# AnyLoc/AnyLoc

Hardware: NVIDIA H100
Metric: images/sec end-to-end DINOv2-VLAD descriptors (higher is better)
Workload: dtype f32-equivalent (tensor-core fp16 3-term split, fp32 accumulate)

## Files before the change

### anyloc_b200/_lib.py

```python
import ctypes as C
import os

import torch

_HERE = os.path.dirname(os.path.abspath(__file__))
LIB_PATH = os.path.join(_HERE, "libanyloc_b200.so")

DIST = {"cosine": 0, "euclidean": 1}
METRIC = {"cosine": 0, "l2": 1}
FACET = {"query": 0, "key": 1, "value": 2, "token": 3}
FFN = {"mlp": 0, "swiglufused": 1}
EPI = {"bias": 0, "bias_split": 1, "gelu_split": 2, "swiglu_split": 3, "ls_resid": 4}
ENGINE = {"auto": 0, "simt": 1, "tc3": 2}
PAIR = {"tf32": 0, "f16": 1, "bf16": 2, "fp8": 3, "f16x1": 4}
ACT_SCALE = 8.0
VIT_VARLEN_MAX_B = 128
PREPROCESS_VARLEN_BATCH = 64
ERR = {"arg": -1, "cuda": -2, "workspace": -3, "unsupported": -4}
PCA = {"cov": 0, "gram": 1, "vt": 2, "sketch": 3}
VLAD_ROUTE_SORTED = 2
KMEANS_SMEM_BYTES = 220 * 1024


class AnylocError(RuntimeError):
    pass


class VitCfg(C.Structure):
    _fields_ = [(n, C.c_int) for n in ("embed_dim", "depth", "num_heads", "ffn_kind", "ffn_hidden", "patch",
                                       "pair_dtype", "num_registers")]


_BLOCK_FIELDS = ["ln1_w", "ln1_b", "qkv_w_hi", "qkv_w_lo", "qkv_b", "proj_w_hi", "proj_w_lo", "proj_b",
                 "ls1", "ln2_w", "ln2_b", "in_w_hi", "in_w_lo", "in_b", "out_w_hi", "out_w_lo", "out_b", "ls2"]


class VitBlock(C.Structure):
    _fields_ = [(n, C.c_void_p) for n in _BLOCK_FIELDS] + \
               [(n, C.c_float) for n in ("qkv_alpha", "proj_alpha", "in_alpha", "out_alpha")]


class VitWeightsStruct(C.Structure):
    _fields_ = [("patch_w_hi", C.c_void_p), ("patch_w_lo", C.c_void_p), ("patch_b", C.c_void_p),
                ("cls_token", C.c_void_p), ("blocks", C.POINTER(VitBlock)), ("patch_alpha", C.c_float),
                ("register_tokens", C.c_void_p)]


class VitTap(C.Structure):
    _fields_ = [("layer", C.c_int), ("facet", C.c_int), ("out", C.c_void_p)]


_SIGS = {
    "anyloc_last_error": (C.c_char_p, []),
    "anyloc_version": (C.c_int, []),
    "anyloc_launch_count": (C.c_longlong, []),
    "anyloc_profile_enable": (C.c_int, [C.c_int]),
    "anyloc_profile_read": (C.c_int, [C.POINTER(C.c_double), C.POINTER(C.c_longlong), C.POINTER(C.c_double)]),
    "anyloc_device_info": (C.c_int, [C.POINTER(C.c_int), C.POINTER(C.c_size_t)]),
    "anyloc_vlad_workspace_bytes": (C.c_size_t, [C.c_int] * 4),
    "anyloc_vlad_generate": (C.c_int, [C.c_void_p, C.c_void_p, C.c_void_p] + [C.c_int] * 7 +
                             [C.c_void_p, C.c_void_p, C.c_void_p, C.c_size_t, C.c_void_p]),
    "anyloc_vlad_prepared_bytes": (C.c_size_t, [C.c_int] * 2),
    "anyloc_vlad_prepare": (C.c_int, [C.c_void_p, C.c_int, C.c_int, C.c_int, C.c_void_p, C.c_size_t, C.c_void_p]),
    "anyloc_vlad_generate_prepared": (C.c_int, [C.c_void_p, C.c_void_p, C.c_void_p, C.c_void_p, C.c_size_t] +
                                      [C.c_int] * 7 + [C.c_void_p, C.c_void_p, C.c_void_p, C.c_size_t, C.c_void_p]),
    "anyloc_vlad_generate_route": (C.c_int, [C.c_int] * 4),
    "anyloc_vlad_sorted_workspace_bytes": (C.c_size_t, [C.c_int] * 4),
    "anyloc_vlad_generate_sorted": (C.c_int, [C.c_void_p, C.c_void_p, C.c_void_p, C.c_void_p, C.c_size_t] +
                                    [C.c_int] * 7 + [C.c_void_p, C.c_void_p, C.c_void_p, C.c_size_t, C.c_void_p]),
    "anyloc_vlad_generate_soft": (C.c_int, [C.c_void_p, C.c_void_p, C.c_void_p] + [C.c_int] * 4 + [C.c_float] +
                                  [C.c_int] * 2 + [C.c_void_p, C.c_void_p, C.c_void_p, C.c_size_t, C.c_void_p]),
    "anyloc_preprocess_u8": (C.c_int, [C.c_void_p] + [C.c_int] * 7 + [C.POINTER(C.c_float)] * 2 +
                             [C.c_void_p, C.c_void_p]),
    "anyloc_preprocess_resize_u8": (C.c_int, [C.c_void_p] + [C.c_int] * 10 + [C.POINTER(C.c_float)] * 2 +
                                    [C.c_void_p, C.c_void_p]),
    "anyloc_preprocess_u8_varlen": (C.c_int, [C.c_int, C.POINTER(C.c_void_p)] + [C.POINTER(C.c_int)] * 4 + [C.c_int] +
                                    [C.POINTER(C.c_int)] * 4 + [C.POINTER(C.c_float)] * 2 +
                                    [C.c_void_p, C.POINTER(C.c_int64), C.c_void_p]),
    "anyloc_pool": (C.c_int, [C.c_void_p, C.c_void_p] + [C.c_int] * 4 + [C.c_float, C.c_int, C.c_void_p, C.c_void_p]),
    "anyloc_vlad_residuals": (C.c_int, [C.c_void_p, C.c_void_p] + [C.c_int] * 4 + [C.c_void_p, C.c_void_p]),
    "anyloc_vlad_from_residuals_workspace_bytes": (C.c_size_t, [C.c_int] * 2),
    "anyloc_vlad_from_residuals": (C.c_int, [C.c_void_p, C.c_void_p, C.c_void_p] + [C.c_int] * 4 +
                                   [C.c_void_p, C.c_void_p, C.c_size_t, C.c_void_p]),
    "anyloc_vlad_assign": (C.c_int, [C.c_void_p, C.c_void_p] + [C.c_int] * 4 +
                           [C.c_void_p, C.c_void_p, C.c_size_t, C.c_void_p]),
    "anyloc_kmeans_workspace_bytes": (C.c_size_t, [C.c_int] * 3),
    "anyloc_kmeans_update": (C.c_int, [C.c_void_p, C.c_void_p, C.c_void_p] + [C.c_int] * 3 +
                             [C.c_void_p, C.c_void_p, C.c_void_p, C.c_size_t, C.c_void_p]),
    "anyloc_kmeans_partition": (C.c_int, [C.c_int64, C.c_int, C.POINTER(C.c_int), C.POINTER(C.c_int64)]),
    "anyloc_kmeans_round_workspace_bytes": (C.c_size_t, [C.c_int64, C.c_int, C.c_int]),
    "anyloc_kmeans_accumulate_round": (C.c_int, [C.c_void_p, C.c_void_p, C.c_int64, C.c_int64, C.c_int64, C.c_int,
                                                 C.c_int, C.c_int, C.c_void_p, C.c_size_t, C.c_void_p]),
    "anyloc_kmeans_finalize": (C.c_int, [C.c_void_p, C.c_int64, C.c_int, C.c_int, C.c_void_p, C.c_void_p, C.c_void_p,
                                         C.c_size_t, C.c_void_p]),
    "anyloc_kmeans_accumulate_round_tiled": (C.c_int, [C.c_void_p, C.c_void_p, C.c_int64, C.c_int64, C.c_int64] +
                                             [C.c_int] * 4 + [C.c_void_p, C.c_size_t, C.c_void_p]),
    "anyloc_kmeans_update_tiled": (C.c_int, [C.c_void_p, C.c_void_p, C.c_void_p, C.c_int64] + [C.c_int] * 3 +
                                   [C.c_void_p, C.c_void_p, C.c_void_p, C.c_size_t, C.c_void_p]),
    "anyloc_topk_workspace_bytes": (C.c_size_t, [C.c_int] * 4),
    "anyloc_topk": (C.c_int, [C.c_void_p, C.c_void_p] + [C.c_int] * 6 +
                    [C.c_void_p, C.c_void_p, C.c_void_p, C.c_size_t, C.c_void_p]),
    "anyloc_index_bytes": (C.c_size_t, [C.c_int64, C.c_int, C.c_int]),
    "anyloc_index_init": (C.c_int, [C.c_void_p, C.c_size_t, C.c_int64, C.c_int, C.c_int, C.c_void_p]),
    "anyloc_index_copy": (C.c_int, [C.c_void_p, C.c_size_t, C.c_int64, C.c_void_p, C.c_size_t, C.c_int64, C.c_int64,
                                    C.c_int, C.c_int, C.c_void_p]),
    "anyloc_index_add": (C.c_int, [C.c_void_p, C.c_size_t, C.c_int64, C.c_int64, C.c_void_p, C.c_int, C.c_int, C.c_int,
                                   C.c_void_p]),
    "anyloc_index_search_workspace_bytes": (C.c_size_t, [C.c_int64, C.c_int, C.c_int, C.c_int]),
    "anyloc_index_search": (C.c_int, [C.c_void_p, C.c_size_t, C.c_int64, C.c_int64, C.c_void_p] + [C.c_int] * 5 +
                            [C.c_void_p, C.c_void_p, C.c_void_p, C.c_size_t, C.c_void_p]),
    "anyloc_index_search_continue": (C.c_int, [C.c_void_p, C.c_size_t] + [C.c_int64] * 5 + [C.c_void_p] +
                                     [C.c_int] * 5 + [C.c_void_p, C.c_void_p, C.c_void_p, C.c_size_t, C.c_void_p]),
    "anyloc_index_split_bytes": (C.c_size_t, [C.c_int64, C.c_int]),
    "anyloc_index_split_init": (C.c_int, [C.c_void_p, C.c_size_t, C.c_int64, C.c_int, C.c_void_p]),
    "anyloc_index_split_copy": (C.c_int, [C.c_void_p, C.c_size_t, C.c_int64, C.c_void_p, C.c_size_t, C.c_int64,
                                          C.c_int64, C.c_int, C.c_void_p]),
    "anyloc_index_split_add": (C.c_int, [C.c_void_p, C.c_size_t, C.c_int64, C.c_void_p, C.c_int64, C.c_void_p, C.c_int,
                                         C.c_int, C.c_void_p]),
    "anyloc_index_split_search_workspace_bytes": (C.c_size_t, [C.c_int64, C.c_int, C.c_int]),
    "anyloc_index_split_stage_bytes": (C.c_size_t, [C.c_int64, C.c_int]),
    "anyloc_index_split_search": (C.c_int, [C.c_void_p, C.c_size_t, C.c_int64, C.c_int64, C.c_void_p] + [C.c_int] * 3 +
                                  [C.c_void_p, C.c_size_t, C.POINTER(C.c_int64), C.c_void_p]),
    "anyloc_index_split_rescore": (C.c_int, [C.c_void_p, C.c_size_t, C.c_int64, C.c_void_p, C.c_int64] + [C.c_int] * 3 +
                                   [C.c_void_p, C.c_size_t, C.c_int64, C.c_void_p, C.c_size_t, C.c_void_p, C.c_void_p,
                                    C.c_void_p]),
    "anyloc_index_split_piece": (C.c_int, [C.c_void_p, C.c_size_t, C.c_int64, C.c_void_p, C.c_size_t, C.c_int64,
                                           C.c_void_p, C.c_int64, C.c_int64, C.c_int, C.c_void_p]),
    "anyloc_allgather_desc": (C.c_int, [C.c_void_p, C.c_void_p, C.c_void_p, C.c_size_t, C.c_int, C.c_void_p]),
    "anyloc_vit_patch_k": (C.c_int, [C.c_int]),
    "anyloc_vit_workspace_bytes": (C.c_size_t, [C.POINTER(VitCfg), C.c_int, C.c_int, C.c_int]),
    "anyloc_vit_extract": (C.c_int, [C.POINTER(VitCfg), C.POINTER(VitWeightsStruct), C.c_void_p,
                                     C.c_int, C.c_int, C.c_int, C.c_void_p, C.c_int, C.c_int, C.c_int,
                                     C.c_int, C.c_void_p, C.c_void_p, C.c_size_t, C.c_int, C.c_void_p]),
    "anyloc_vit_varlen_workspace_bytes": (C.c_size_t, [C.POINTER(VitCfg), C.c_int, C.POINTER(C.c_int32)]),
    "anyloc_vit_extract_varlen": (C.c_int, [C.POINTER(VitCfg), C.POINTER(VitWeightsStruct), C.c_int,
                                            C.POINTER(C.c_void_p), C.POINTER(C.c_int32), C.POINTER(C.c_void_p),
                                            C.c_int, C.c_int, C.c_int, C.c_int, C.c_void_p, C.c_void_p, C.c_size_t,
                                            C.c_int, C.c_void_p]),
    "anyloc_vit_taps_workspace_bytes": (C.c_size_t, [C.POINTER(VitCfg), C.c_int, C.c_int, C.c_int, C.POINTER(VitTap),
                                                     C.c_int]),
    "anyloc_vit_extract_taps": (C.c_int, [C.POINTER(VitCfg), C.POINTER(VitWeightsStruct), C.c_void_p, C.c_int, C.c_int,
                                          C.c_int, C.c_void_p, C.POINTER(VitTap), C.c_int, C.c_int, C.c_int,
                                          C.c_void_p, C.c_size_t, C.c_int, C.c_void_p]),
    "anyloc_vit_taps_varlen_workspace_bytes": (C.c_size_t, [C.POINTER(VitCfg), C.c_int, C.POINTER(C.c_int32),
                                                            C.POINTER(VitTap), C.c_int]),
    "anyloc_vit_extract_taps_varlen": (C.c_int, [C.POINTER(VitCfg), C.POINTER(VitWeightsStruct), C.c_int,
                                                 C.POINTER(C.c_void_p), C.POINTER(C.c_int32), C.POINTER(C.c_void_p),
                                                 C.POINTER(VitTap), C.c_int, C.c_int, C.c_int, C.c_void_p, C.c_size_t,
                                                 C.c_int, C.c_void_p]),
    "anyloc_gemm_nt": (C.c_int, [C.c_void_p, C.c_void_p, C.c_int, C.c_void_p, C.c_void_p, C.c_int,
                                 C.c_int, C.c_int, C.c_int, C.c_int, C.c_float, C.c_int, C.c_void_p, C.c_void_p,
                                 C.c_void_p, C.c_void_p, C.c_void_p, C.c_int, C.c_int, C.c_int, C.c_void_p]),
    "anyloc_gemm_tc_last_staged": (C.c_int, []),
    "anyloc_split_tf32": (C.c_int, [C.c_void_p, C.c_void_p, C.c_void_p, C.c_size_t, C.c_void_p]),
    "anyloc_split_f16": (C.c_int, [C.c_void_p, C.c_void_p, C.c_void_p, C.c_size_t, C.c_float, C.c_void_p]),
    "anyloc_split_bf16": (C.c_int, [C.c_void_p, C.c_void_p, C.c_size_t, C.c_void_p]),
    "anyloc_layernorm_split": (C.c_int, [C.c_void_p, C.c_void_p, C.c_void_p, C.c_int, C.c_int, C.c_float,
                                         C.c_void_p, C.c_void_p, C.c_int, C.c_void_p]),
    "anyloc_fp8_scale": (C.c_float, [C.c_float]),
    "anyloc_quantize_fp8_rows": (C.c_int, [C.c_void_p, C.c_int, C.c_int, C.c_void_p, C.c_void_p, C.c_void_p]),
    "anyloc_quantize_fp8_tensor": (C.c_int, [C.c_void_p, C.c_void_p, C.c_size_t, C.POINTER(C.c_float), C.c_void_p]),
    "anyloc_attention": (C.c_int, [C.c_void_p, C.c_void_p, C.c_int, C.c_int, C.c_int, C.c_int, C.c_void_p,
                                   C.c_void_p, C.c_int, C.c_int, C.c_void_p]),
    "anyloc_attention_varlen": (C.c_int, [C.c_void_p, C.c_void_p, C.c_int, C.POINTER(C.c_int32),
                                          C.POINTER(C.c_int32), C.c_int, C.c_int, C.c_void_p, C.c_void_p, C.c_int,
                                          C.c_void_p]),
    "anyloc_l2_normalize_rows": (C.c_int, [C.c_void_p, C.c_int64, C.c_int, C.c_int64, C.c_void_p, C.c_void_p]),
    "anyloc_pca_colsum_workspace_bytes": (C.c_size_t, [C.c_int64, C.c_int]),
    "anyloc_pca_colsum": (C.c_int, [C.c_void_p, C.c_int64, C.c_int64, C.c_int, C.c_void_p, C.c_void_p, C.c_size_t,
                                    C.c_void_p]),
    "anyloc_pca_accumulate": (C.c_int, [C.c_int, C.c_void_p, C.c_int64, C.c_int64, C.c_int, C.c_void_p, C.c_void_p,
                                        C.c_int64, C.c_int, C.c_void_p, C.c_int64, C.c_void_p]),
    "anyloc_pca_mirror": (C.c_int, [C.c_void_p, C.c_int, C.c_int64, C.c_void_p]),
}
EXPORTS = sorted(_SIGS)

_lib = None


def load():
    global _lib
    if _lib is None:
        if not os.path.isfile(LIB_PATH):
            raise AnylocError(
                f"{LIB_PATH} is missing -- build it with `python -m anyloc_b200.build` "
                "(anyloc_b200 has no CPU fallback)")
        lib = C.CDLL(LIB_PATH)
        for name, (res, args) in _SIGS.items():
            fn = getattr(lib, name)
            fn.restype, fn.argtypes = res, args
        _lib = lib
    return _lib


def last_error():
    return load().anyloc_last_error().decode()


def check(rc, what):
    if rc != 0:
        raise AnylocError(f"{what} failed (rc={rc}): {last_error()}")


def require_cuda(device=None):
    if not torch.cuda.is_available():
        raise AnylocError("anyloc_b200 needs a CUDA device (sm_90a); there is no CPU fallback")
    load()
    dev = torch.device("cuda" if device is None else device)
    if dev.type != "cuda":
        raise AnylocError(f"anyloc_b200 runs on CUDA devices only (got device={device!r}); no CPU fallback")
    if dev.index is None:
        dev = torch.device("cuda", torch.cuda.current_device())
    return dev


def stream_ptr():
    return C.c_void_p(torch.cuda.current_stream().cuda_stream)


def ptr(t):
    if t is None:
        return C.c_void_p(0)
    assert t.is_cuda and t.is_contiguous(), "device-contiguous tensor required"
    return C.c_void_p(t.data_ptr())


class _WorkspacePool:

    def __init__(self):
        self._bufs = {}

    def get(self, device, nbytes, tag="default"):
        key = (device.index, tag)
        buf = self._bufs.get(key)
        if buf is None or buf.numel() < nbytes:
            self._bufs.pop(key, None)
            buf = None
            buf = torch.empty(int(nbytes), dtype=torch.uint8, device=device)
            self._bufs[key] = buf
        return buf

    def clear(self):
        self._bufs.clear()


workspaces = _WorkspacePool()

PROF_CATEGORIES = ["gemm_tc", "gemm_simt", "attention", "layernorm", "vit_misc", "vlad", "topk"]


def profile_enable(on=True):
    check(load().anyloc_profile_enable(int(bool(on))), "profile_enable")


def profile_read():
    n = len(PROF_CATEGORIES)
    ms, groups, work = (C.c_double * n)(), (C.c_longlong * n)(), (C.c_double * n)()
    check(load().anyloc_profile_read(ms, groups, work), "profile_read")
    return {c: (ms[i], groups[i], work[i]) for i, c in enumerate(PROF_CATEGORIES)}


def launch_count():
    return int(load().anyloc_launch_count())
```

### anyloc_b200/csrc/gemm_tc.cu

```cuda
#include <cuda.h>
#include <stdlib.h>
#include "epilogue.cuh"
#include "tc_common.cuh"

namespace anyloc {

namespace tc {

constexpr int BM = 128, BN = 128;
constexpr int KSTEPS = 4;
constexpr int A_BYTES = BM * 128;
constexpr int B_BYTES = BN * 128;
constexpr int THREADS = 384;
constexpr int STG_BYTES = 8192;

template <bool LO, bool STG = LO> struct Cfg {
  static constexpr int STAGE_BYTES = (LO ? 2 : 1) * (A_BYTES + B_BYTES);
  static constexpr int B_OFF = (LO ? 2 : 1) * A_BYTES;
  static constexpr int STAGES = LO ? 3 : 6;
  static constexpr int BAR_OFF = STAGES * STAGE_BYTES;
  static constexpr int SMEM_BYTES = BAR_OFF + 256 + 1024 ;
  static constexpr bool STAGED = STG;
  static constexpr int STG_OFF = BAR_OFF + 1024;
  static constexpr int SMEM_BYTES_STAGED = STG_OFF + 4 * STG_BYTES + 1024 ;
};
constexpr int BAND_N = 16;
constexpr int CHUNK_KB_TF32 = 2;
constexpr int CHUNK_KB_F16 = 8;
constexpr int CHUNK_KB_COARSE = 32;
constexpr int CHUNK_KB_FP8 = 1;

__device__ __forceinline__ void tile_coords(int tile, int num_m, int num_n, int band_n, int& m_blk, int& n_blk) {
  const int per_band = num_m * band_n;
  const int band = tile / per_band, r = tile - band * per_band;
  const int w = min(band_n, num_n - band * band_n);
  m_blk = r / w;
  n_blk = band * band_n + (r - m_blk * w);
}

template <int OUT>
__device__ __forceinline__ void split_put2(const EpiParams& ep, size_t o, float a, float b) {
  typedef typename Fmt<OUT>::T T;
  put2<OUT>(reinterpret_cast<T*>(ep.out), reinterpret_cast<T*>(ep.out_lo), o, a, b);
}
template <int FMT = ANYLOC_PAIR_TF32>
__device__ __forceinline__ void store_split2(const EpiParams& ep, size_t o, float a, float b) {
  if constexpr (!Fmt<FMT>::LO) split_put2<Fmt<FMT>::OUT>(ep, o, a, b);
  else if (ep.out_fmt != ANYLOC_PAIR_TF32) split_put2<ANYLOC_PAIR_F16>(ep, o, a, b);
  else split_put2<ANYLOC_PAIR_TF32>(ep, o, a, b);
}

template <int FMT = ANYLOC_PAIR_TF32>
__device__ __forceinline__ void epi_pair(const EpiParams& ep, int m, int n, int N, float v0, float v1) {
  const int mode = ep.mode;
  if (mode < 0) return;
  if (mode == ANYLOC_EPI_SWIGLU_SPLIT) {
    epi_store_pair<FMT>(ep, m, n, v0, v1);
    return;
  }
  if (n + 1 >= N || (ep.ldo & 1)) {
    epi_store1<FMT>(ep, m, n, v0);
    if (n + 1 < N) epi_store1<FMT>(ep, m, n + 1, v1);
    return;
  }
  const float al = ep.alpha;
  float2 b = make_float2(0.f, 0.f);
  if (ep.bias) b = __ldg(reinterpret_cast<const float2*>(ep.bias + n));
  const float x0 = v0 * al + b.x, x1 = v1 * al + b.y;
  const size_t o = (size_t)m * ep.ldo + n;
  if (mode == ANYLOC_EPI_BIAS) {
    *reinterpret_cast<float2*>(ep.out + o) = make_float2(x0, x1);
  } else if (mode == ANYLOC_EPI_LS_RESID) {
    const float2 g = __ldg(reinterpret_cast<const float2*>(ep.gamma + n));
    const float2 r = *reinterpret_cast<const float2*>(ep.resid + o);
    *reinterpret_cast<float2*>(ep.out + o) = make_float2(r.x + g.x * x0, r.y + g.y * x1);
  } else if (mode == ANYLOC_EPI_GELU_SPLIT) {
    store_split2<FMT>(ep, o, gelu_erf(x0), gelu_erf(x1));
  } else {
    store_split2<FMT>(ep, o, x0, x1);
  }
}

template <int FMT = ANYLOC_PAIR_TF32>
__device__ __forceinline__ void epilogue_pairs(const EpiParams& ep, int r0, int nq, int M, int N, const float* sum) {
#pragma unroll
  for (int j = 0; j < 16; ++j) {
    const int n = nq + j * 8;
    if (n >= N) continue;
    if (r0 < M) epi_pair<FMT>(ep, r0, n, N, sum[4 * j], sum[4 * j + 1]);
    if (r0 + 8 < M) epi_pair<FMT>(ep, r0 + 8, n, N, sum[4 * j + 2], sum[4 * j + 3]);
  }
}

__device__ __forceinline__ void epilogue_regs_batched(const EpiParams& ep, int r0, int nq, int M, int N, const float* sum) {
  const int mode = ep.mode;
  if (mode < 0) return;
  const int n0 = nq & ~(BN - 1);
  const bool swiglu = mode == ANYLOC_EPI_SWIGLU_SPLIT, resid = mode == ANYLOC_EPI_LS_RESID;
  if (n0 + BN > N || (!swiglu && (ep.ldo & 1))) {
    epilogue_pairs(ep, r0, nq, M, N, sum);
    return;
  }
  const bool row0 = r0 < M, row1 = r0 + 8 < M;
  const size_t o0 = (size_t)r0 * ep.ldo, o1 = (size_t)(r0 + 8) * ep.ldo;
  const float al = ep.alpha;
#pragma unroll
  for (int j0 = 0; j0 < 16; j0 += 2) {
    float2 b[2], g[2], ra[2], rb[2];
#pragma unroll
    for (int jj = 0; jj < 2; ++jj) {
      const int n = nq + (j0 + jj) * 8;
      b[jj] = ep.bias ? __ldg(reinterpret_cast<const float2*>(ep.bias + n)) : make_float2(0.f, 0.f);
      if (resid) {
        g[jj] = __ldg(reinterpret_cast<const float2*>(ep.gamma + n));
        if (row0) ra[jj] = *reinterpret_cast<const float2*>(ep.resid + o0 + n);
        if (row1) rb[jj] = *reinterpret_cast<const float2*>(ep.resid + o1 + n);
      }
    }
#pragma unroll
    for (int jj = 0; jj < 2; ++jj) {
      const int j = j0 + jj, n = nq + j * 8;
#pragma unroll
      for (int h = 0; h < 2; ++h) {
        if (!(h ? row1 : row0)) continue;
        const float v0 = sum[4 * j + 2 * h], v1 = sum[4 * j + 2 * h + 1];
        const size_t ro = h ? o1 : o0;
        if (swiglu) {
          const float x1 = v0 * al + b[jj].x, x2 = v1 * al + b[jj].y;
          epi_store_split(ep, ro + (n >> 1), silu(x1) * x2);
          continue;
        }
        const float x0 = v0 * al + b[jj].x, x1 = v1 * al + b[jj].y;
        const size_t o = ro + n;
        if (mode == ANYLOC_EPI_BIAS) {
          *reinterpret_cast<float2*>(ep.out + o) = make_float2(x0, x1);
        } else if (resid) {
          const float2 r = h ? rb[jj] : ra[jj];
          *reinterpret_cast<float2*>(ep.out + o) = make_float2(r.x + g[jj].x * x0, r.y + g[jj].y * x1);
        } else if (mode == ANYLOC_EPI_GELU_SPLIT) {
          store_split2(ep, o, gelu_erf(x0), gelu_erf(x1));
        } else {
          store_split2(ep, o, x0, x1);
        }
      }
    }
  }
}

constexpr int OUT_F32 = -1;
constexpr int STG_HALF = STG_BYTES / 2;
constexpr int STG_ROWS = 64;

template <int OUT> constexpr bool stage_lo() {
  if constexpr (OUT == OUT_F32) return false;
  else return Fmt<OUT>::LO;
}
template <int OUT> constexpr int stage_esz() {
  if constexpr (OUT == OUT_F32) return 4;
  else return (int)sizeof(typename Fmt<OUT>::T);
}
template <int OUT>
struct StageFmt {
  static constexpr bool LO = stage_lo<OUT>();
  static constexpr int ESZ = stage_esz<OUT>();
  static constexpr int ROW_BYTES = STG_BYTES / STG_ROWS / (LO ? 2 : 1);
  static constexpr int COLS = ROW_BYTES / ESZ;
  static constexpr uint32_t SWZ = ROW_BYTES == 128 ? 7 : 3;
};

template <int OUT>
__device__ __forceinline__ uint32_t stg_off(int row, int b) {
  const uint32_t o = (uint32_t)(row * StageFmt<OUT>::ROW_BYTES + b);
  return o ^ (((o >> 7) & StageFmt<OUT>::SWZ) << 4);
}

__device__ __forceinline__ float2 ldg_col_pair(const float* p, int n, int N) {
  if (n + 1 < N) return __ldg(reinterpret_cast<const float2*>(p + n));
  return make_float2(n < N ? __ldg(p + n) : 0.f, 0.f);
}

__device__ __forceinline__ void resid_load(const CUtensorMap* tm, uint8_t* buf, uint64_t* bar, int oc, int m0) {
  mbar_expect_tx(smem_u32(bar), STG_BYTES);
  tma_load_2d(smem_u32(buf), tm, smem_u32(bar), oc, m0);
}

template <int OUT, bool SWIGLU, bool RESID>
__device__ __forceinline__ void epilogue_staged(const EpiParams& ep, const CUtensorMap* tm_out, const CUtensorMap* tm_lo,
                                                const CUtensorMap* tm_resid, uint8_t* stg, uint64_t* rbar,
                                                uint32_t& rphase, uint32_t& cnt, int wg, int t, int m0, int n0, int N,
                                                const float* sum) {
  using F = StageFmt<OUT>;
  constexpr int ACC = SWIGLU ? 2 * F::COLS : F::COLS;
  constexpr int JS = ACC / 8;
  const int lane = t & 31, q = lane & 3, row = (t >> 5) * 16 + (lane >> 2);
  const int n_out = SWIGLU ? N >> 1 : N;
  const int oc_base = SWIGLU ? n0 >> 1 : n0;
  const bool gelu = ep.mode == ANYLOC_EPI_GELU_SPLIT;
  const float al = ep.alpha;
#pragma unroll
  for (int s = 0; s < BN / ACC; ++s) {
    const int oc0 = oc_base + s * F::COLS;
    if (oc0 >= n_out) break;
    const uint32_t b = cnt & 1;
    uint8_t* buf = stg + b * STG_BYTES;
    if (RESID) { mbar_wait(smem_u32(rbar + b), (rphase >> b) & 1); rphase ^= 1u << b; }
#pragma unroll
    for (int jj = 0; jj < JS; ++jj) {
      const int j = s * JS + jj, n = n0 + j * 8 + 2 * q;
      const float2 bb = ep.bias ? ldg_col_pair(ep.bias, n, N) : make_float2(0.f, 0.f);
      float2 g;
      if (RESID) g = ldg_col_pair(ep.gamma, n, N);
#pragma unroll
      for (int h = 0; h < 2; ++h) {
        const int r = row + 8 * h;
        const float x0 = sum[4 * j + 2 * h] * al + bb.x, x1 = sum[4 * j + 2 * h + 1] * al + bb.y;
        if constexpr (SWIGLU) {
          typedef typename Fmt<OUT>::T E;
          const float v = silu(x0) * x1;
          const uint32_t o = stg_off<OUT>(r, (4 * jj + q) * F::ESZ);
          E hi, lo;
          Fmt<OUT>::split1(v, hi, lo);
          *reinterpret_cast<E*>(buf + o) = hi;
          if constexpr (F::LO) *reinterpret_cast<E*>(buf + STG_HALF + o) = lo;
          continue;
        }
        const uint32_t o = stg_off<OUT>(r, (8 * jj + 2 * q) * F::ESZ);
        if constexpr (OUT == OUT_F32) {
          float2* p = reinterpret_cast<float2*>(buf + o);
          if (RESID) {
            const float2 rr = *p;
            *p = make_float2(rr.x + g.x * x0, rr.y + g.y * x1);
          } else {
            *p = make_float2(x0, x1);
          }
        } else {
          typedef typename Fmt<OUT>::W2 W;
          const float y0 = gelu ? gelu_erf(x0) : x0, y1 = gelu ? gelu_erf(x1) : x1;
          W hi, lo;
          Fmt<OUT>::split2(y0, y1, hi, lo);
          *reinterpret_cast<W*>(buf + o) = hi;
          if constexpr (F::LO) *reinterpret_cast<W*>(buf + STG_HALF + o) = lo;
        }
      }
    }
    fence_proxy_async_smem();
    if (t == 0) bulk_wait_read<0>();
    if (wg == 1) named_bar_sync<1>(128);
    else named_bar_sync<2>(128);
    if (t == 0) {
      tma_store_2d(tm_out, smem_u32(buf), oc0, m0);
      if (F::LO) tma_store_2d(tm_lo, smem_u32(buf + STG_HALF), oc0, m0);
      bulk_commit();
      if (RESID && s + 2 < BN / ACC && oc0 + 2 * F::COLS < n_out) {
        bulk_wait_read<0>();
        resid_load(tm_resid, buf, rbar + b, oc0 + 2 * F::COLS, m0);
      }
    }
    ++cnt;
  }
}

template <int FMT, int LOM>
__global__ void __launch_bounds__(THREADS, 1)
gemm_tc3_kernel(const __grid_constant__ CUtensorMap tm_a_hi, const __grid_constant__ CUtensorMap tm_a_lo,
                const __grid_constant__ CUtensorMap tm_b_hi, const __grid_constant__ CUtensorMap tm_b_lo,
                const __grid_constant__ CUtensorMap tm_out, const __grid_constant__ CUtensorMap tm_out_lo,
                const __grid_constant__ CUtensorMap tm_resid, int staged,
                int M, int N, int K, int band_n, int chunk_kb, EpiParams ep) {
  constexpr bool LO = LOM != 0, has_a_lo = (LOM & 1) != 0, has_b_lo = (LOM & 2) != 0;
  static_assert(LOM == 0 || Fmt<FMT>::LO, "lo operands belong to the pair formats");
  using C = Cfg<LO, LO || !Fmt<FMT>::LO>;
  if (ep.gate != nullptr && *reinterpret_cast<const volatile int*>(ep.gate) == 0) return;
  extern __shared__ uint8_t smem_raw[];
  uint8_t* smem = reinterpret_cast<uint8_t*>((reinterpret_cast<uintptr_t>(smem_raw) + 1023) & ~(uintptr_t)1023);
  uint64_t* full_bar = reinterpret_cast<uint64_t*>(smem + C::BAR_OFF);
  uint64_t* empty_bar = full_bar + C::STAGES;
  uint64_t* resid_bar = empty_bar + C::STAGES;

  const int wg = threadIdx.x >> 7;
  const int num_m = (M + BM - 1) / BM, num_n = (N + BN - 1) / BN;
  const int num_tiles = num_m * num_n;
  constexpr int BKE = 128 / (int)sizeof(typename Fmt<FMT>::T);
  const int num_k = (K + BKE - 1) / BKE;

  if (threadIdx.x == 0) {
    asm volatile("prefetch.tensormap [%0];" ::"l"(&tm_a_hi) : "memory");
    asm volatile("prefetch.tensormap [%0];" ::"l"(&tm_b_hi) : "memory");
    for (int s = 0; s < C::STAGES; ++s) { mbar_init(smem_u32(full_bar + s), 1); mbar_init(smem_u32(empty_bar + s), 2); }
    if (C::STAGED)
      for (int i = 0; i < 4; ++i) mbar_init(smem_u32(resid_bar + i), 1);
    asm volatile("fence.mbarrier_init.release.cluster;" ::: "memory");
  }
  __syncthreads();

  if (wg == 0) {
    if (threadIdx.x == 0) {
      const uint32_t tx_bytes = A_BYTES * (1 + ((LO && has_a_lo) ? 1 : 0)) + B_BYTES * (1 + ((LO && has_b_lo) ? 1 : 0));
      int stage = 0; uint32_t phase = 0;
      for (int tile = blockIdx.x; tile < num_tiles; tile += gridDim.x) {
        int mb, nb; tile_coords(tile, num_m, num_n, band_n, mb, nb);
        const int m0 = mb * BM, n0 = nb * BN;
        for (int kb = 0; kb < num_k; ++kb) {
          mbar_wait(smem_u32(empty_bar + stage), phase ^ 1);
          const uint32_t fb = smem_u32(full_bar + stage);
          mbar_expect_tx(fb, tx_bytes);
          const uint32_t sbase = smem_u32(smem + stage * C::STAGE_BYTES);
          tma_load_2d(sbase, &tm_a_hi, fb, kb * BKE, m0);
          if (LO && has_a_lo) tma_load_2d(sbase + A_BYTES, &tm_a_lo, fb, kb * BKE, m0);
          tma_load_2d(sbase + C::B_OFF, &tm_b_hi, fb, kb * BKE, n0);
          if (LO && has_b_lo) tma_load_2d(sbase + C::B_OFF + B_BYTES, &tm_b_lo, fb, kb * BKE, n0);
          if (++stage == C::STAGES) { stage = 0; phase ^= 1; }
        }
      }
    }
    return;
  }

  const int t = threadIdx.x & 127, warp = t >> 5, lane = t & 31;
  const uint32_t a_sub = (uint32_t)(wg - 1) * 64 * 128;
  uint8_t* stg = smem + C::STG_OFF + (wg - 1) * 2 * STG_BYTES;
  uint64_t* rbar = resid_bar + (wg - 1) * 2;
  const int mode = ep.mode;
  staged = C::STAGED && staged;
  const bool resid_staged = staged && mode == ANYLOC_EPI_LS_RESID;
  uint32_t stg_cnt = 0, rphase = 0;
  int stage = 0; uint32_t phase = 0;
  for (int tile = blockIdx.x; tile < num_tiles; tile += gridDim.x) {
    int mb, nb; tile_coords(tile, num_m, num_n, band_n, mb, nb);
    const int m0 = mb * BM + (wg - 1) * 64, n0 = nb * BN;
    float sum[64], acc[64];
#pragma unroll
    for (int j = 0; j < 64; ++j) { sum[j] = 0.f; acc[j] = 0.f; }
    int prev_stage = -1;
    for (int kb0 = 0; kb0 < num_k; kb0 += chunk_kb) {
      const int kb1 = min(num_k, kb0 + chunk_kb);
      if (resid_staged && kb1 == num_k && t == 0 && m0 < M) {
        bulk_wait_read<0>();
        for (int i = 0; i < 2; ++i) {
          const uint32_t b = (stg_cnt + i) & 1;
          const int oc = n0 + i * StageFmt<OUT_F32>::COLS;
          if (oc < N) resid_load(&tm_resid, stg + b * STG_BYTES, rbar + b, oc, m0);
        }
      }
      for (int kb = kb0; kb < kb1; ++kb) {
        mbar_wait(smem_u32(full_bar + stage), phase);
        const uint32_t sbase = smem_u32(smem + stage * C::STAGE_BYTES);
        const uint64_t a_hi = make_desc(sbase + a_sub), a_lo = make_desc(sbase + A_BYTES + a_sub);
        const uint64_t b_hi = make_desc(sbase + C::B_OFF), b_lo = make_desc(sbase + C::B_OFF + B_BYTES);
        wgmma_fence();
#pragma unroll
        for (int k = 0; k < KSTEPS; ++k) {
          const uint64_t adv = (uint64_t)((k * 32) >> 4);
          wgmma_m64n128<FMT>(acc, a_hi + adv, b_hi + adv, (kb != kb0 || k != 0) ? 1u : 0u);
          if (has_a_lo) wgmma_m64n128<FMT>(acc, a_lo + adv, b_hi + adv, 1u);
          if (has_b_lo) wgmma_m64n128<FMT>(acc, a_hi + adv, b_lo + adv, 1u);
        }
        wgmma_commit();
        wgmma_wait<1>();
        if (prev_stage >= 0 && t == 0) mbar_arrive(smem_u32(empty_bar + prev_stage));
        prev_stage = stage;
        if (++stage == C::STAGES) { stage = 0; phase ^= 1; }
      }
      wgmma_wait<0>();
      fence_regs<64>(acc);
#pragma unroll
      for (int j = 0; j < 64; ++j) sum[j] += acc[j];
    }
    if (t == 0) mbar_arrive(smem_u32(empty_bar + prev_stage));
    if (mode < 0 || m0 >= M) continue;
    if constexpr (FMT == ANYLOC_PAIR_FP8) {
      const int r = m0 + warp * 16 + (lane >> 2);
      const float s0 = r < M ? __ldg(ep.row_scale + r) : 0.f, s1 = r + 8 < M ? __ldg(ep.row_scale + r + 8) : 0.f;
#pragma unroll
      for (int j = 0; j < 16; ++j) { sum[4 * j] *= s0; sum[4 * j + 1] *= s0; sum[4 * j + 2] *= s1; sum[4 * j + 3] *= s1; }
    }
    if constexpr (!C::STAGED) {
      epilogue_regs_batched(ep, m0 + warp * 16 + (lane >> 2), n0 + 2 * (lane & 3), M, N, sum);
      continue;
    }
    if (!staged) {
      epilogue_pairs<FMT>(ep, m0 + warp * 16 + (lane >> 2), n0 + 2 * (lane & 3), M, N, sum);
      continue;
    }
#define ANYLOC_EPI_STAGED(OUT_, SWIGLU_, RESID_)                                                                    \
  epilogue_staged<OUT_, SWIGLU_, RESID_>(ep, &tm_out, &tm_out_lo, &tm_resid, stg, rbar, rphase, stg_cnt, wg, t, m0,  \
                                         n0, N, sum)
    if (mode == ANYLOC_EPI_BIAS) ANYLOC_EPI_STAGED(OUT_F32, false, false);
    else if (mode == ANYLOC_EPI_LS_RESID) ANYLOC_EPI_STAGED(OUT_F32, false, true);
    else if constexpr (!Fmt<FMT>::LO) {
      if (mode == ANYLOC_EPI_SWIGLU_SPLIT) ANYLOC_EPI_STAGED(Fmt<FMT>::OUT, true, false);
      else ANYLOC_EPI_STAGED(Fmt<FMT>::OUT, false, false);
    } else if (mode == ANYLOC_EPI_SWIGLU_SPLIT) {
      if (ep.out_fmt != ANYLOC_PAIR_TF32) ANYLOC_EPI_STAGED(ANYLOC_PAIR_F16, true, false);
      else ANYLOC_EPI_STAGED(ANYLOC_PAIR_TF32, true, false);
    } else {
      if (ep.out_fmt != ANYLOC_PAIR_TF32) ANYLOC_EPI_STAGED(ANYLOC_PAIR_F16, false, false);
      else ANYLOC_EPI_STAGED(ANYLOC_PAIR_TF32, false, false);
    }
#undef ANYLOC_EPI_STAGED
  }
  if (staged && t == 0) bulk_wait<0>();
}

typedef CUresult (*EncodeTiledFn)(CUtensorMap*, CUtensorMapDataType, cuuint32_t, void*, const cuuint64_t*,
                                  const cuuint64_t*, const cuuint32_t*, const cuuint32_t*, CUtensorMapInterleave,
                                  CUtensorMapSwizzle, CUtensorMapL2promotion, CUtensorMapFloatOOBfill);

static EncodeTiledFn get_encode() {
  static EncodeTiledFn fn = nullptr;
  if (!fn) {
    void* p = nullptr;
    cudaDriverEntryPointQueryResult q;
    if (cudaGetDriverEntryPoint("cuTensorMapEncodeTiled", &p, cudaEnableDefault, &q) != cudaSuccess ||
        q != cudaDriverEntryPointSuccess)
      return nullptr;
    fn = (EncodeTiledFn)p;
  }
  return fn;
}

static CUtensorMapDataType map_dtype(int fmt) {
  switch (fmt) {
    case ANYLOC_PAIR_FP8: return CU_TENSOR_MAP_DATA_TYPE_UINT8;
    case ANYLOC_PAIR_BF16: return CU_TENSOR_MAP_DATA_TYPE_BFLOAT16;
    case ANYLOC_PAIR_F16: case ANYLOC_PAIR_F16X1: return CU_TENSOR_MAP_DATA_TYPE_FLOAT16;
    default: return CU_TENSOR_MAP_DATA_TYPE_FLOAT32;
  }
}

int make_map(CUtensorMap* map, const void* ptr, int rows, int K, int ld, int box_rows, int fmt) {
  EncodeTiledFn enc = get_encode();
  if (!enc) { set_error("gemm_tc: cuTensorMapEncodeTiled unavailable"); return ANYLOC_ERR_CUDA; }
  const int esz = format_info(fmt).esz;
  cuuint64_t dims[2] = {(cuuint64_t)K, (cuuint64_t)rows};
  cuuint64_t strides[1] = {(cuuint64_t)ld * esz};
  cuuint32_t box[2] = {(cuuint32_t)(128 / esz), (cuuint32_t)box_rows};
  cuuint32_t estr[2] = {1, 1};
  CUresult r = enc(map, map_dtype(fmt), 2, (void*)ptr, dims, strides, box, estr, CU_TENSOR_MAP_INTERLEAVE_NONE, CU_TENSOR_MAP_SWIZZLE_128B,
                   CU_TENSOR_MAP_L2_PROMOTION_L2_256B, CU_TENSOR_MAP_FLOAT_OOB_FILL_NONE);
  if (r != CUDA_SUCCESS) { set_error("gemm_tc: cuTensorMapEncodeTiled failed (%d) rows=%d K=%d ld=%d", (int)r, rows, K, ld); return ANYLOC_ERR_CUDA; }
  return ANYLOC_OK;
}

int make_map_3d16(CUtensorMap* map, const void* ptr, int imgs, int rows, int cols, int box_rows, int fmt) {
  EncodeTiledFn enc = get_encode();
  if (!enc) { set_error("tensor map: cuTensorMapEncodeTiled unavailable"); return ANYLOC_ERR_CUDA; }
  cuuint64_t dims[3] = {(cuuint64_t)cols, (cuuint64_t)rows, (cuuint64_t)imgs};
  cuuint64_t strides[2] = {(cuuint64_t)cols * 2, (cuuint64_t)rows * cols * 2};
  cuuint32_t box[3] = {64, (cuuint32_t)box_rows, 1};
  cuuint32_t estr[3] = {1, 1, 1};
  CUresult r = enc(map, map_dtype(fmt), 3, (void*)ptr, dims,
                   strides, box, estr, CU_TENSOR_MAP_INTERLEAVE_NONE, CU_TENSOR_MAP_SWIZZLE_128B,
                   CU_TENSOR_MAP_L2_PROMOTION_L2_256B, CU_TENSOR_MAP_FLOAT_OOB_FILL_NONE);
  if (r != CUDA_SUCCESS) { set_error("tensor map: cuTensorMapEncodeTiled failed (%d) imgs=%d rows=%d cols=%d", (int)r, imgs, rows, cols); return ANYLOC_ERR_CUDA; }
  return ANYLOC_OK;
}

static int make_out_map(CUtensorMap* map, const void* ptr, int rows, int cols, int ld, int fmt, int box_cols) {
  const int esz = format_info(fmt).esz;
  EncodeTiledFn enc = get_encode();
  if (!enc) { set_error("gemm_tc: cuTensorMapEncodeTiled unavailable"); return ANYLOC_ERR_CUDA; }
  cuuint64_t dims[2] = {(cuuint64_t)cols, (cuuint64_t)rows};
  cuuint64_t strides[1] = {(cuuint64_t)ld * esz};
  cuuint32_t box[2] = {(cuuint32_t)box_cols, (cuuint32_t)STG_ROWS};
  cuuint32_t estr[2] = {1, 1};
  CUresult r = enc(map, map_dtype(fmt), 2, (void*)ptr, dims, strides, box, estr, CU_TENSOR_MAP_INTERLEAVE_NONE,
                   box_cols * esz == 128 ? CU_TENSOR_MAP_SWIZZLE_128B : CU_TENSOR_MAP_SWIZZLE_64B,
                   CU_TENSOR_MAP_L2_PROMOTION_L2_256B, CU_TENSOR_MAP_FLOAT_OOB_FILL_NONE);
  if (r != CUDA_SUCCESS) { set_error("gemm_tc: cuTensorMapEncodeTiled failed (%d) for the output: rows=%d cols=%d ld=%d", (int)r, rows, cols, ld); return ANYLOC_ERR_CUDA; }
  return ANYLOC_OK;
}

static int make_epi_maps(const EpiParams& ep, int out, int M, int N, CUtensorMap* m_out, CUtensorMap* m_lo,
                         CUtensorMap* m_resid, bool* staged) {
  memset(m_out, 0, sizeof(*m_out)); memset(m_lo, 0, sizeof(*m_lo)); memset(m_resid, 0, sizeof(*m_resid));
  const bool split = ep.mode == ANYLOC_EPI_BIAS_SPLIT || ep.mode == ANYLOC_EPI_GELU_SPLIT ||
                     ep.mode == ANYLOC_EPI_SWIGLU_SPLIT;
  const int fmt = split ? out : ANYLOC_PAIR_TF32;
  const FormatInfo& f = format_info(fmt);
  const int esz = f.esz;
  const int n_out = ep.mode == ANYLOC_EPI_SWIGLU_SPLIT ? N / 2 : N;
  *staged = ep.mode >= 0 && ((long long)ep.ldo * esz) % 16 == 0 && ((long long)n_out * esz) % 16 == 0;
  if (!*staged) return ANYLOC_OK;
  const bool lo = split && f.lo;
  const int cols = STG_BYTES / STG_ROWS / (lo ? 2 : 1) / esz;
  int rc;
  if ((rc = make_out_map(m_out, ep.out, M, n_out, ep.ldo, fmt, cols))) return rc;
  if (lo && (rc = make_out_map(m_lo, ep.out_lo, M, n_out, ep.ldo, fmt, cols))) return rc;
  if (ep.mode == ANYLOC_EPI_LS_RESID && (rc = make_out_map(m_resid, ep.resid, M, n_out, ep.ldo, fmt, cols))) return rc;
  return ANYLOC_OK;
}

}

bool gemm_tc_supported(const void* a_hi, const void* a_lo, int lda, const void* b_hi, const void* b_lo, int ldb,
                       int M, int N, int K, const EpiParams& ep, int fmt) {
  auto al16 = [](const void* p) { return (reinterpret_cast<uintptr_t>(p) & 15) == 0; };
  const int q = 16 / format_info(fmt).esz;
  if (M < 1 || N < 1 || K < q) return false;
  if ((K % q) || (lda % q) || (ldb % q)) return false;
  if (!al16(a_hi) || !al16(b_hi) || (a_lo && !al16(a_lo)) || (b_lo && !al16(b_lo))) return false;
  if (!al16(ep.out) || (ep.out_lo && !al16(ep.out_lo)) || (ep.resid && !al16(ep.resid))) return false;
  if (ep.bias && !al16(ep.bias)) return false;
  if (ep.gamma && !al16(ep.gamma)) return false;
  return true;
}

static thread_local int g_last_staged = -1;

template <int FMT, int LOM>
static int launch_impl(const void* a_hi, const void* a_lo, int lda, const void* b_hi, const void* b_lo, int ldb, int M,
                       int N, int K, const EpiParams& ep, int chunk, cudaStream_t st) {
  using namespace tc;
  constexpr bool LO = LOM != 0;
  using CF = Cfg<LO, LO || !Fmt<FMT>::LO>;
  static_assert(CF::SMEM_BYTES_STAGED <= 232448, "GEMM over H100's shared-memory opt-in");
  CUtensorMap ma_hi, ma_lo, mb_hi, mb_lo;
  int rc;
  if ((rc = make_map(&ma_hi, a_hi, M, K, lda, BM, FMT))) return rc;
  if ((rc = make_map(&ma_lo, a_lo ? a_lo : a_hi, M, K, lda, BM, FMT))) return rc;
  if ((rc = make_map(&mb_hi, b_hi, N, K, ldb, BN, FMT))) return rc;
  if ((rc = make_map(&mb_lo, b_lo ? b_lo : b_hi, N, K, ldb, BN, FMT))) return rc;
  CUtensorMap mo, mo_lo, mr;
  bool staged = false;
  memset(&mo, 0, sizeof(mo)); memset(&mo_lo, 0, sizeof(mo_lo)); memset(&mr, 0, sizeof(mr));
  const int out = Fmt<FMT>::LO ? (ep.out_fmt != ANYLOC_PAIR_TF32 ? ANYLOC_PAIR_F16 : ANYLOC_PAIR_TF32) : Fmt<FMT>::OUT;
  if (CF::STAGED && ep.gate == nullptr && (rc = make_epi_maps(ep, out, M, N, &mo, &mo_lo, &mr, &staged))) return rc;
  const int smem = staged ? CF::SMEM_BYTES_STAGED : CF::SMEM_BYTES;
  g_last_staged = staged ? 1 : 0;
  static unsigned long long attr_seen = 0;
  if (first_use_on_this_device(&attr_seen)) {
    ANYLOC_CHECK_CUDA(cudaFuncSetAttribute(gemm_tc3_kernel<FMT, LOM>, cudaFuncAttributeMaxDynamicSharedMemorySize,
                                           CF::STAGED ? CF::SMEM_BYTES_STAGED : CF::SMEM_BYTES));
  }
  const int tiles = cdiv(M, BM) * cdiv(N, BN);
  const int grid = std::min(tiles, device_sm_count());
  gemm_tc3_kernel<FMT, LOM><<<grid, THREADS, smem, st>>>(
      ma_hi, ma_lo, mb_hi, mb_lo, mo, mo_lo, mr, staged ? 1 : 0, M, N, K, std::min(BAND_N, cdiv(N, BN)), chunk, ep);
  ANYLOC_CHECK_LAUNCH();
  return ANYLOC_OK;
}

static int gemm_chunk_env() {
  static int chunk_env = -1;
  if (chunk_env < 0) { const char* e = getenv("ANYLOC_GEMM_CHUNK"); chunk_env = e ? atoi(e) : 0; }
  return chunk_env;
}

int gemm_tc_launch(const void* a_hi, const void* a_lo, int lda, const void* b_hi, const void* b_lo, int ldb, int M,
                   int N, int K, const EpiParams& ep_in, int fmt, cudaStream_t st) {
  const int chunk_env = gemm_chunk_env();
  EpiParams ep = ep_in;
  switch (fmt) {
    case ANYLOC_PAIR_BF16:
      return launch_impl<ANYLOC_PAIR_BF16, 0>(a_hi, nullptr, lda, b_hi, nullptr, ldb, M, N, K, ep, tc::CHUNK_KB_F16, st);
    case ANYLOC_PAIR_F16X1:
      return launch_impl<ANYLOC_PAIR_F16X1, 0>(a_hi, nullptr, lda, b_hi, nullptr, ldb, M, N, K, ep, tc::CHUNK_KB_F16,
                                               st);
    case ANYLOC_PAIR_FP8:
      ep.row_scale = static_cast<const float*>(a_lo);
      return launch_impl<ANYLOC_PAIR_FP8, 0>(a_hi, nullptr, lda, b_hi, nullptr, ldb, M, N, K, ep,
                                             chunk_env > 0 ? chunk_env : tc::CHUNK_KB_FP8, st);
    default: break;
  }
  static int skip_epi = -1;
  if (skip_epi < 0) { const char* e = getenv("ANYLOC_GEMM_DEBUG_SKIP_EPI"); skip_epi = e ? atoi(e) : 0; }
  if (skip_epi && ((skip_epi >> ep_in.mode) & 1)) ep.mode = -1;
  const bool f16 = fmt == ANYLOC_PAIR_F16;
  const int lom = (a_lo ? 1 : 0) | (b_lo ? 2 : 0);
  const int chunk = lom == 0 ? (f16 ? tc::CHUNK_KB_COARSE : tc::CHUNK_KB_TF32)
                             : chunk_env > 0 ? chunk_env : (f16 ? tc::CHUNK_KB_F16 : tc::CHUNK_KB_TF32);
#define ANYLOC_GEMM_LAUNCH(FMT_, LOM_) launch_impl<FMT_, LOM_>(a_hi, a_lo, lda, b_hi, b_lo, ldb, M, N, K, ep, chunk, st)
  switch (lom + (f16 ? 4 : 0)) {
    case 0: return ANYLOC_GEMM_LAUNCH(ANYLOC_PAIR_TF32, 0);
    case 1: return ANYLOC_GEMM_LAUNCH(ANYLOC_PAIR_TF32, 1);
    case 2: return ANYLOC_GEMM_LAUNCH(ANYLOC_PAIR_TF32, 2);
    case 3: return ANYLOC_GEMM_LAUNCH(ANYLOC_PAIR_TF32, 3);
    case 4: return ANYLOC_GEMM_LAUNCH(ANYLOC_PAIR_F16, 0);
    case 5: return ANYLOC_GEMM_LAUNCH(ANYLOC_PAIR_F16, 1);
    case 6: return ANYLOC_GEMM_LAUNCH(ANYLOC_PAIR_F16, 2);
    default: return ANYLOC_GEMM_LAUNCH(ANYLOC_PAIR_F16, 3);
  }
#undef ANYLOC_GEMM_LAUNCH
}

}

extern "C" int anyloc_gemm_tc_last_staged(void) { return anyloc::g_last_staged; }
```

### anyloc_b200/csrc/tc_common.cuh

```cuda
#pragma once
#include <cuda.h>
#include "formats.cuh"

namespace anyloc {
namespace tc {

__device__ __forceinline__ uint32_t smem_u32(const void* p) { return (uint32_t)__cvta_generic_to_shared(p); }

__device__ __forceinline__ void mbar_init(uint32_t bar, uint32_t count) {
  asm volatile("mbarrier.init.shared::cta.b64 [%0], %1;" ::"r"(bar), "r"(count));
}
__device__ __forceinline__ void mbar_expect_tx(uint32_t bar, uint32_t bytes) {
  asm volatile("mbarrier.arrive.expect_tx.shared::cta.b64 _, [%0], %1;" ::"r"(bar), "r"(bytes) : "memory");
}
__device__ __forceinline__ void mbar_arrive(uint32_t bar) {
  asm volatile("mbarrier.arrive.shared::cta.b64 _, [%0];" ::"r"(bar) : "memory");
}
__device__ __forceinline__ void mbar_wait(uint32_t bar, uint32_t parity) {
  uint32_t done = 0;
  long long t0 = 0;
  for (uint32_t it = 0; !done; ++it) {
    asm volatile(
        "{\n\t.reg .pred p;\n\t"
        "mbarrier.try_wait.parity.shared::cta.b64 p, [%1], %2;\n\t"
        "selp.u32 %0, 1, 0, p;\n\t}"
        : "=r"(done) : "r"(bar), "r"(parity) : "memory");
    if (!done && (it & 0x3ff) == 0x3ff) {
      long long now = clock64();
      if (t0 == 0) t0 = now;
      else if (now - t0 > 8000000000LL) __trap();
    }
  }
}
__device__ __forceinline__ void tma_load_2d(uint32_t dst, const CUtensorMap* map, uint32_t bar, int c0, int c1) {
  asm volatile(
      "cp.async.bulk.tensor.2d.shared::cluster.global.mbarrier::complete_tx::bytes [%0], [%1, {%3, %4}], [%2];"
      ::"r"(dst), "l"(map), "r"(bar), "r"(c0), "r"(c1) : "memory");
}

__device__ __forceinline__ void tma_store_2d(const CUtensorMap* map, uint32_t src, int c0, int c1) {
  asm volatile("cp.async.bulk.tensor.2d.global.shared::cta.bulk_group [%0, {%2, %3}], [%1];"
               ::"l"(map), "r"(src), "r"(c0), "r"(c1) : "memory");
}
__device__ __forceinline__ void bulk_commit() { asm volatile("cp.async.bulk.commit_group;" ::: "memory"); }
template <int N>
__device__ __forceinline__ void bulk_wait_read() { asm volatile("cp.async.bulk.wait_group.read %0;" ::"n"(N) : "memory"); }
template <int N>
__device__ __forceinline__ void bulk_wait() { asm volatile("cp.async.bulk.wait_group %0;" ::"n"(N) : "memory"); }
__device__ __forceinline__ void fence_proxy_async_smem() { asm volatile("fence.proxy.async.shared::cta;" ::: "memory"); }
template <int ID>
__device__ __forceinline__ void named_bar_sync(int count) {
  asm volatile("bar.sync %0, %1;" ::"n"(ID), "r"(count) : "memory");
}

__device__ __forceinline__ uint64_t make_desc(uint32_t saddr) {
  uint64_t d = 0;
  d |= (uint64_t)((saddr & 0x3FFFF) >> 4);
  d |= (uint64_t)1 << 16;
  d |= (uint64_t)(1024 >> 4) << 32;
  d |= (uint64_t)1 << 62;
  return d;
}

__device__ __forceinline__ void wgmma_fence() { asm volatile("wgmma.fence.sync.aligned;" ::: "memory"); }
__device__ __forceinline__ void wgmma_commit() { asm volatile("wgmma.commit_group.sync.aligned;" ::: "memory"); }
template <int N>
__device__ __forceinline__ void wgmma_wait() { asm volatile("wgmma.wait_group.sync.aligned %0;" ::"n"(N) : "memory"); }
template <int R>
__device__ __forceinline__ void fence_regs(float* d) {
#pragma unroll
  for (int i = 0; i < R; ++i) asm volatile("" : "+f"(d[i])::"memory");
}

#define ANYLOC_WG_D64                                                                                               \
  "+f"(d[0]), "+f"(d[1]), "+f"(d[2]), "+f"(d[3]), "+f"(d[4]), "+f"(d[5]), "+f"(d[6]), "+f"(d[7]), "+f"(d[8]),       \
      "+f"(d[9]), "+f"(d[10]), "+f"(d[11]), "+f"(d[12]), "+f"(d[13]), "+f"(d[14]), "+f"(d[15]), "+f"(d[16]),        \
      "+f"(d[17]), "+f"(d[18]), "+f"(d[19]), "+f"(d[20]), "+f"(d[21]), "+f"(d[22]), "+f"(d[23]), "+f"(d[24]),       \
      "+f"(d[25]), "+f"(d[26]), "+f"(d[27]), "+f"(d[28]), "+f"(d[29]), "+f"(d[30]), "+f"(d[31]), "+f"(d[32]),       \
      "+f"(d[33]), "+f"(d[34]), "+f"(d[35]), "+f"(d[36]), "+f"(d[37]), "+f"(d[38]), "+f"(d[39]), "+f"(d[40]),       \
      "+f"(d[41]), "+f"(d[42]), "+f"(d[43]), "+f"(d[44]), "+f"(d[45]), "+f"(d[46]), "+f"(d[47]), "+f"(d[48]),       \
      "+f"(d[49]), "+f"(d[50]), "+f"(d[51]), "+f"(d[52]), "+f"(d[53]), "+f"(d[54]), "+f"(d[55]), "+f"(d[56]),       \
      "+f"(d[57]), "+f"(d[58]), "+f"(d[59]), "+f"(d[60]), "+f"(d[61]), "+f"(d[62]), "+f"(d[63])
#define ANYLOC_WG_D64_STR                                                                                           \
  "{%0, %1, %2, %3, %4, %5, %6, %7, %8, %9, %10, %11, %12, %13, %14, %15, %16, %17, %18, %19, %20, %21, %22, %23, " \
  "%24, %25, %26, %27, %28, %29, %30, %31, %32, %33, %34, %35, %36, %37, %38, %39, %40, %41, %42, %43, %44, %45, "  \
  "%46, %47, %48, %49, %50, %51, %52, %53, %54, %55, %56, %57, %58, %59, %60, %61, %62, %63}"
#define ANYLOC_WG_M64N128(SHAPE_TYPES, TAIL)                                                                        \
  asm volatile("{\n\t.reg .pred p;\n\tsetp.ne.b32 p, %66, 0;\n\t"                                                 \
               "wgmma.mma_async.sync.aligned.m64n128" SHAPE_TYPES " " ANYLOC_WG_D64_STR ", %64, %65, p, 1, 1" TAIL     \
               ";\n\t}"                                                                                              \
               : ANYLOC_WG_D64 : "l"(adesc), "l"(bdesc), "r"(scale_d))

template <int FMT>
__device__ __forceinline__ void wgmma_m64n128(float* d, uint64_t adesc, uint64_t bdesc, uint32_t scale_d) {
  if constexpr (FMT == ANYLOC_PAIR_TF32) ANYLOC_WG_M64N128("k8.f32.tf32.tf32", "");
  else if constexpr (FMT == ANYLOC_PAIR_FP8) ANYLOC_WG_M64N128("k32.f32.e4m3.e4m3", "");
  else if constexpr (FMT == ANYLOC_PAIR_BF16) ANYLOC_WG_M64N128("k16.f32.bf16.bf16", ", 0, 0");
  else ANYLOC_WG_M64N128("k16.f32.f16.f16", ", 0, 0");
}
#undef ANYLOC_WG_M64N128
#undef ANYLOC_WG_D64
#undef ANYLOC_WG_D64_STR

__device__ __forceinline__ void tma_load_3d(uint32_t dst, const CUtensorMap* map, uint32_t bar, int c0, int c1, int c2) {
  asm volatile(
      "cp.async.bulk.tensor.3d.shared::cluster.global.mbarrier::complete_tx::bytes [%0], [%1, {%3, %4, %5}], [%2];"
      ::"r"(dst), "l"(map), "r"(bar), "r"(c0), "r"(c1), "r"(c2) : "memory");
}

template <int N> __device__ __forceinline__ void setmaxnreg_dec() { asm volatile("setmaxnreg.dec.sync.aligned.u32 %0;" ::"n"(N)); }
template <int N> __device__ __forceinline__ void setmaxnreg_inc() { asm volatile("setmaxnreg.inc.sync.aligned.u32 %0;" ::"n"(N)); }

__device__ __forceinline__ uint64_t make_desc_mn(uint32_t saddr) {
  uint64_t d = 0;
  d |= (uint64_t)((saddr & 0x3FFFF) >> 4);
  d |= (uint64_t)(1024 >> 4) << 16;
  d |= (uint64_t)(1024 >> 4) << 32;
  d |= (uint64_t)1 << 62;
  return d;
}

#define ANYLOC_WG_D32                                                                                               \
  "+f"(d[0]), "+f"(d[1]), "+f"(d[2]), "+f"(d[3]), "+f"(d[4]), "+f"(d[5]), "+f"(d[6]), "+f"(d[7]), "+f"(d[8]),       \
      "+f"(d[9]), "+f"(d[10]), "+f"(d[11]), "+f"(d[12]), "+f"(d[13]), "+f"(d[14]), "+f"(d[15]), "+f"(d[16]),        \
      "+f"(d[17]), "+f"(d[18]), "+f"(d[19]), "+f"(d[20]), "+f"(d[21]), "+f"(d[22]), "+f"(d[23]), "+f"(d[24]),       \
      "+f"(d[25]), "+f"(d[26]), "+f"(d[27]), "+f"(d[28]), "+f"(d[29]), "+f"(d[30]), "+f"(d[31])
#define ANYLOC_WG_D32_STR                                                                                           \
  "{%0, %1, %2, %3, %4, %5, %6, %7, %8, %9, %10, %11, %12, %13, %14, %15, %16, %17, %18, %19, %20, %21, %22, %23, " \
  "%24, %25, %26, %27, %28, %29, %30, %31}"

template <int FMT>
__device__ __forceinline__ void wgmma_m64n64_ss(float* d, uint64_t adesc, uint64_t bdesc, uint32_t scale_d) {
  if constexpr (FMT == ANYLOC_PAIR_BF16)
    asm volatile("{\n\t.reg .pred p;\n\tsetp.ne.b32 p, %34, 0;\n\t"
                 "wgmma.mma_async.sync.aligned.m64n64k16.f32.bf16.bf16 " ANYLOC_WG_D32_STR ", %32, %33, p, 1, 1, 0, 0;\n\t}"
                 : ANYLOC_WG_D32 : "l"(adesc), "l"(bdesc), "r"(scale_d));
  else
    asm volatile("{\n\t.reg .pred p;\n\tsetp.ne.b32 p, %34, 0;\n\t"
                 "wgmma.mma_async.sync.aligned.m64n64k16.f32.f16.f16 " ANYLOC_WG_D32_STR ", %32, %33, p, 1, 1, 0, 0;\n\t}"
                 : ANYLOC_WG_D32 : "l"(adesc), "l"(bdesc), "r"(scale_d));
}

template <int FMT>
__device__ __forceinline__ void wgmma_m64n64_rs_tb(float* d, const uint32_t* a, uint64_t bdesc, uint32_t scale_d) {
  if constexpr (FMT == ANYLOC_PAIR_BF16)
    asm volatile("{\n\t.reg .pred p;\n\tsetp.ne.b32 p, %37, 0;\n\t"
                 "wgmma.mma_async.sync.aligned.m64n64k16.f32.bf16.bf16 " ANYLOC_WG_D32_STR
                 ", {%32, %33, %34, %35}, %36, p, 1, 1, 1;\n\t}"
                 : ANYLOC_WG_D32 : "r"(a[0]), "r"(a[1]), "r"(a[2]), "r"(a[3]), "l"(bdesc), "r"(scale_d));
  else
    asm volatile("{\n\t.reg .pred p;\n\tsetp.ne.b32 p, %37, 0;\n\t"
                 "wgmma.mma_async.sync.aligned.m64n64k16.f32.f16.f16 " ANYLOC_WG_D32_STR
                 ", {%32, %33, %34, %35}, %36, p, 1, 1, 1;\n\t}"
                 : ANYLOC_WG_D32 : "r"(a[0]), "r"(a[1]), "r"(a[2]), "r"(a[3]), "l"(bdesc), "r"(scale_d));
}
#undef ANYLOC_WG_D32
#undef ANYLOC_WG_D32_STR

int make_map(CUtensorMap* map, const void* ptr, int rows, int K, int ld, int box_rows, int fmt);
int make_map_3d16(CUtensorMap* map, const void* ptr, int imgs, int rows, int cols, int box_rows, int fmt);

}
}
```

### include/anyloc_b200.h

```cpp
#ifndef ANYLOC_B200_H
#define ANYLOC_B200_H

#include <stddef.h>
#include <stdint.h>

#ifdef __cplusplus
extern "C" {
#endif

#define ANYLOC_OK 0
#define ANYLOC_ERR_ARG (-1)
#define ANYLOC_ERR_CUDA (-2)
#define ANYLOC_ERR_WORKSPACE (-3)
#define ANYLOC_ERR_UNSUPPORTED (-4)

#define ANYLOC_DIST_COSINE 0
#define ANYLOC_DIST_EUCLIDEAN 1
#define ANYLOC_METRIC_IP 0
#define ANYLOC_METRIC_L2 1
#define ANYLOC_FACET_QUERY 0
#define ANYLOC_FACET_KEY 1
#define ANYLOC_FACET_VALUE 2
#define ANYLOC_FACET_TOKEN 3
#define ANYLOC_FFN_MLP 0
#define ANYLOC_FFN_SWIGLU 1

#define ANYLOC_EPI_BIAS 0
#define ANYLOC_EPI_BIAS_SPLIT 1
#define ANYLOC_EPI_GELU_SPLIT 2
#define ANYLOC_EPI_SWIGLU_SPLIT 3
#define ANYLOC_EPI_LS_RESID 4
#define ANYLOC_PAIR_TF32 0
#define ANYLOC_PAIR_F16 1
#define ANYLOC_PAIR_BF16 2
#define ANYLOC_PAIR_FP8 3
#define ANYLOC_PAIR_F16X1 4
#define ANYLOC_GEMM_AUTO 0
#define ANYLOC_GEMM_SIMT 1
#define ANYLOC_GEMM_TC3 2

const char* anyloc_last_error(void);
int anyloc_version(void);
int anyloc_device_info(int* sm_count, size_t* smem_optin_bytes);

#define ANYLOC_PROF_CATEGORIES 7
long long anyloc_launch_count(void);
int anyloc_profile_enable(int on);
int anyloc_profile_read(double* ms, long long* groups, double* work);

size_t anyloc_vlad_workspace_bytes(int B, int N, int D, int K);
int anyloc_vlad_generate(const float* feats, const int32_t* n_valid, const float* centers,
                         int B, int N, int D, int K, int dist_mode, int norm_descs, int intra_norm,
                         float* vlad, int32_t* labels, void* ws, size_t ws_bytes, void* stream);
size_t anyloc_vlad_prepared_bytes(int D, int K);
int anyloc_vlad_prepare(const float* centers, int D, int K, int dist_mode, void* prepared, size_t prepared_bytes,
                        void* stream);
int anyloc_vlad_generate_prepared(const float* feats, const int32_t* n_valid, const float* centers, void* prepared,
                                  size_t prepared_bytes, int B, int N, int D, int K, int dist_mode, int norm_descs,
                                  int intra_norm, float* vlad, int32_t* labels, void* ws, size_t ws_bytes, void* stream);
#define ANYLOC_VLAD_ROUTE_ACC3 0
#define ANYLOC_VLAD_ROUTE_ACC2 1
#define ANYLOC_VLAD_ROUTE_SORTED 2
int anyloc_vlad_generate_route(int B, int N, int D, int K);
size_t anyloc_vlad_sorted_workspace_bytes(int B, int N, int D, int K);
int anyloc_vlad_generate_sorted(const float* feats, const int32_t* n_valid, const float* centers, void* prepared,
                                size_t prepared_bytes, int B, int N, int D, int K, int dist_mode, int norm_descs,
                                int intra_norm, float* vlad, int32_t* labels, void* ws, size_t ws_bytes, void* stream);
int anyloc_vlad_generate_soft(const float* feats, const int32_t* n_valid, const float* centers,
                              int B, int N, int D, int K, float soft_temp, int norm_descs, int intra_norm,
                              float* vlad, float* assign, void* ws, size_t ws_bytes, void* stream);
int anyloc_vlad_residuals(const float* feats, const float* centers, int N, int D, int K, int norm_descs,
                          float* out, void* stream);
size_t anyloc_vlad_from_residuals_workspace_bytes(int D, int K);
int anyloc_vlad_from_residuals(const float* resid, const int32_t* labels, const float* assign, int N, int D, int K,
                               int intra_norm, float* vlad, void* ws, size_t ws_bytes, void* stream);
int anyloc_vlad_assign(const float* feats, const float* centers, int R, int D, int K, int dist_mode,
                       int32_t* labels, void* ws, size_t ws_bytes, void* stream);
size_t anyloc_kmeans_workspace_bytes(int R, int D, int K);
int anyloc_kmeans_update(const float* x, const int32_t* labels, const float* old_centers, int R, int D,
                         int K, float* new_centers, float* err_out, void* ws, size_t ws_bytes,
                         void* stream);
int anyloc_kmeans_partition(int64_t R, int D, int* chunks, int64_t* rows_per);
size_t anyloc_kmeans_round_workspace_bytes(int64_t R, int D, int K);
int anyloc_kmeans_accumulate_round(const float* x, const int32_t* labels, int64_t R, int64_t round_rows,
                                   int64_t piece_rows, int D, int K, int resume, void* ws, size_t ws_bytes,
                                   void* stream);
int anyloc_kmeans_finalize(const float* old_centers, int64_t R, int D, int K, float* new_centers, float* err_out,
                           void* ws, size_t ws_bytes, void* stream);
int anyloc_kmeans_accumulate_round_tiled(const float* x, const int32_t* labels, int64_t R, int64_t round_rows,
                                         int64_t piece_rows, int D, int K, int k_tile, int resume, void* ws,
                                         size_t ws_bytes, void* stream);
int anyloc_kmeans_update_tiled(const float* x, const int32_t* labels, const float* old_centers, int64_t R, int D,
                               int K, int k_tile, float* new_centers, float* err_out, void* ws, size_t ws_bytes,
                               void* stream);

size_t anyloc_topk_workspace_bytes(int n_db, int n_q, int Dv, int k);
int anyloc_topk(const float* db, const float* qu, int n_db, int n_q, int Dv, int k, int metric,
                int normalize, float* dist, int64_t* idx, void* ws, size_t ws_bytes, void* stream);

size_t anyloc_index_bytes(int64_t capacity, int Dv, int normalize);
int anyloc_index_init(void* index, size_t index_bytes, int64_t capacity, int Dv, int normalize, void* stream);
int anyloc_index_copy(void* dst, size_t dst_bytes, int64_t dst_capacity, const void* src, size_t src_bytes,
                      int64_t src_capacity, int64_t n_rows, int Dv, int normalize, void* stream);
int anyloc_index_add(void* index, size_t index_bytes, int64_t capacity, int64_t row_offset, const float* rows,
                     int n_rows, int Dv, int normalize, void* stream);
size_t anyloc_index_search_workspace_bytes(int64_t n_db, int n_q, int Dv, int normalize);
int anyloc_index_search(const void* index, size_t index_bytes, int64_t capacity, int64_t n_db, const float* qu,
                        int n_q, int Dv, int k, int metric, int normalize, float* dist, int64_t* idx, void* ws,
                        size_t ws_bytes, void* stream);
int anyloc_index_search_continue(const void* index, size_t index_bytes, int64_t capacity, int64_t first,
                                 int64_t n_rows, int64_t row0, int64_t n_total, const float* qu, int n_q, int Dv, int k,
                                 int metric, int normalize, float* dist, int64_t* idx, void* ws, size_t ws_bytes,
                                 void* stream);
size_t anyloc_index_split_bytes(int64_t capacity, int Dv);
int anyloc_index_split_init(void* index, size_t index_bytes, int64_t capacity, int Dv, void* stream);
int anyloc_index_split_copy(void* dst, size_t dst_bytes, int64_t dst_capacity, const void* src, size_t src_bytes,
                            int64_t src_capacity, int64_t n_rows, int Dv, void* stream);
int anyloc_index_split_add(void* index, size_t index_bytes, int64_t capacity, void* lo, int64_t row_offset,
                           const float* rows, int n_rows, int Dv, void* stream);
size_t anyloc_index_split_search_workspace_bytes(int64_t n_db, int n_q, int Dv);
size_t anyloc_index_split_stage_bytes(int64_t rows, int Dv);
int anyloc_index_split_search(const void* index, size_t index_bytes, int64_t capacity, int64_t n_db, const float* qu,
                              int n_q, int Dv, int k, void* ws, size_t ws_bytes, int64_t* counts, void* stream);
int anyloc_index_split_rescore(const void* index, size_t index_bytes, int64_t capacity, const void* lo, int64_t n_db,
                               int n_q, int Dv, int k, void* ws, size_t ws_bytes, int64_t n_unique, void* stage,
                               size_t stage_bytes, float* dist, int64_t* idx, void* stream);
int anyloc_index_split_piece(void* dst, size_t dst_bytes, int64_t dst_capacity, const void* index, size_t index_bytes,
                             int64_t capacity, const void* lo, int64_t first, int64_t n_rows, int Dv, void* stream);

int anyloc_allgather_desc(void* nccl_comm, const float* local, float* all, size_t n_loc, int Dv, void* stream);

typedef struct {
  int embed_dim;
  int depth;
  int num_heads;
  int ffn_kind;
  int ffn_hidden;
  int patch;
  int pair_dtype;
  int num_registers;
} AnylocVitCfg;

typedef struct {
  const float *ln1_w, *ln1_b;
  const void *qkv_w_hi, *qkv_w_lo; const float *qkv_b;
  const void *proj_w_hi, *proj_w_lo; const float *proj_b;
  const float *ls1;
  const float *ln2_w, *ln2_b;
  const void *in_w_hi, *in_w_lo; const float *in_b;
  const void *out_w_hi, *out_w_lo; const float *out_b;
  const float *ls2;
  float qkv_alpha, proj_alpha, in_alpha, out_alpha;
} AnylocVitBlock;

typedef struct {
  const void *patch_w_hi, *patch_w_lo;
  const float *patch_b;
  const float *cls_token;
  const AnylocVitBlock* blocks;
  float patch_alpha;
  const float *register_tokens;
} AnylocVitWeights;

int anyloc_vit_patch_k(int patch);
size_t anyloc_vit_workspace_bytes(const AnylocVitCfg* cfg, int B, int H, int W);
int anyloc_vit_extract(const AnylocVitCfg* cfg, const AnylocVitWeights* w_host, const float* img,
                       int B, int H, int W, const float* pos_embed, int layer, int facet,
                       int use_cls, int norm_descs, float* out, void* ws, size_t ws_bytes,
                       int gemm_engine, void* stream);

#define ANYLOC_VIT_VARLEN_MAX_B 128
size_t anyloc_vit_varlen_workspace_bytes(const AnylocVitCfg* cfg, int B, const int32_t* hw);
int anyloc_vit_extract_varlen(const AnylocVitCfg* cfg, const AnylocVitWeights* w_host, int B, const float* const* img,
                              const int32_t* hw, const float* const* pos_embed, int layer, int facet, int use_cls,
                              int norm_descs, float* out, void* ws, size_t ws_bytes, int gemm_engine, void* stream);

typedef struct {
  int layer;
  int facet;
  float* out;
} AnylocVitTap;
size_t anyloc_vit_taps_workspace_bytes(const AnylocVitCfg* cfg, int B, int H, int W, const AnylocVitTap* taps_host,
                                       int n_taps);
int anyloc_vit_extract_taps(const AnylocVitCfg* cfg, const AnylocVitWeights* w_host, const float* img, int B, int H,
                            int W, const float* pos_embed, const AnylocVitTap* taps_host, int n_taps, int use_cls,
                            int norm_descs, void* ws, size_t ws_bytes, int gemm_engine, void* stream);
size_t anyloc_vit_taps_varlen_workspace_bytes(const AnylocVitCfg* cfg, int B, const int32_t* hw,
                                              const AnylocVitTap* taps_host, int n_taps);
int anyloc_vit_extract_taps_varlen(const AnylocVitCfg* cfg, const AnylocVitWeights* w_host, int B,
                                   const float* const* img, const int32_t* hw, const float* const* pos_embed,
                                   const AnylocVitTap* taps_host, int n_taps, int use_cls, int norm_descs, void* ws,
                                   size_t ws_bytes, int gemm_engine, void* stream);

int anyloc_gemm_nt(const void* a_hi, const void* a_lo, int lda, const void* b_hi, const void* b_lo,
                   int ldb, int M, int N, int K, int in_dtype, float alpha, int epilogue, const float* bias,
                   const float* gamma, const float* resid, void* out, void* out_lo, int ldo, int out_dtype,
                   int engine, void* stream);
int anyloc_gemm_tc_last_staged(void);
int anyloc_split_tf32(const float* x, float* hi, float* lo, size_t n, void* stream);
int anyloc_split_f16(const float* x, void* hi, void* lo, size_t n, float scale, void* stream);
int anyloc_split_bf16(const float* x, void* y, size_t n, void* stream);
int anyloc_layernorm_split(const float* x, const float* w, const float* b, int M, int D, float eps,
                           void* y_hi, void* y_lo, int out_dtype, void* stream);
float anyloc_fp8_scale(float amax);
int anyloc_quantize_fp8_rows(const void* x, int M, int K, void* q, float* scales, void* stream);
int anyloc_quantize_fp8_tensor(const float* x, void* q, size_t n, float* scale_host, void* stream);
int anyloc_attention(const float* qkv_hi, const float* qkv_lo, int B, int T, int D, int heads,
                     void* o_hi, void* o_lo, int out_dtype, int engine, void* stream);
int anyloc_attention_varlen(const void* qkv_hi, const void* qkv_lo, int n, const int32_t* row0, const int32_t* len,
                            int D, int heads, void* o_hi, void* o_lo, int fmt, void* stream);
int anyloc_l2_normalize_rows(const float* x, int64_t rows, int D, int64_t ld_in, float* y, void* stream);

size_t anyloc_pca_colsum_workspace_bytes(int64_t rows, int cols);
int anyloc_pca_colsum(const float* x, int64_t ld, int64_t rows, int cols, double* sum, void* ws, size_t ws_bytes,
                      void* stream);
#define ANYLOC_PCA_COV 0
#define ANYLOC_PCA_GRAM 1
#define ANYLOC_PCA_VT 2
#define ANYLOC_PCA_SKETCH 3
int anyloc_pca_accumulate(int mode, const float* x, int64_t ld, int64_t rows, int cols, const double* mu,
                          const double* u, int64_t ld_u, int k, double* out, int64_t ld_out, void* stream);
int anyloc_pca_mirror(double* a, int m, int64_t ld, void* stream);

#define ANYLOC_POOL_AVG 0
#define ANYLOC_POOL_MAX 1
#define ANYLOC_POOL_GEM 2
int anyloc_pool(const float* feats, const int32_t* n_valid, int B, int N, int D, int mode, float gem_p,
                int gem_use_abs, float* out, void* stream);

int anyloc_preprocess_u8(const uint8_t* img, int B, int H, int W, int top, int left, int Hc, int Wc,
                         const float* mean3, const float* std3, float* out, void* stream);
int anyloc_preprocess_resize_u8(const uint8_t* img, int B, int H, int W, int Hr, int Wr, int interpolation, int top,
                                int left, int Hc, int Wc, const float* mean3, const float* std3, float* out,
                                void* stream);
#define ANYLOC_PREPROCESS_VARLEN_BATCH 64
int anyloc_preprocess_u8_varlen(int n, const uint8_t* const* imgs, const int* H, const int* W, const int* Hr,
                                const int* Wr, int interpolation, const int* top, const int* left, const int* Hc,
                                const int* Wc, const float* mean3, const float* std3, float* out,
                                const int64_t* out_offset, void* stream);

#ifdef __cplusplus
}
#endif
#endif
```

Before: 179.1.

## Add 192-column wgmma tiles for 3-term GEMMs with wave-count selection

Adds a BN=192 tile variant of the warp-specialized 3-term TC GEMM. It uses m64n192 wgmma, a 64-byte K block with 64B swizzle, 4 stages and setmaxnreg register rebalancing. The variant is chosen when a wave-count model predicts fewer waves than 128-column tiles. It also rasters a final M tail of 64 rows or fewer as half-tiles placed after the main grid, and consumer warpgroups with no rows skip the MMA work. The aim is better SM wave quantization and B-operand reuse for ViT GEMMs, at the cost of more register pressure, shallower K blocks and a new heuristic. A force/query API is added for testing.

```diff
diff --git a/anyloc_b200/_lib.py b/anyloc_b200/_lib.py
--- a/anyloc_b200/_lib.py
+++ b/anyloc_b200/_lib.py
@@ -152,6 +152,8 @@
                                  C.c_int, C.c_int, C.c_int, C.c_int, C.c_float, C.c_int, C.c_void_p, C.c_void_p,
                                  C.c_void_p, C.c_void_p, C.c_void_p, C.c_int, C.c_int, C.c_int, C.c_void_p]),
     "anyloc_gemm_tc_last_staged": (C.c_int, []),
+    "anyloc_gemm_tc_last_bn": (C.c_int, []),
+    "anyloc_gemm_tc_force_bn": (C.c_int, [C.c_int]),
     "anyloc_split_tf32": (C.c_int, [C.c_void_p, C.c_void_p, C.c_void_p, C.c_size_t, C.c_void_p]),
     "anyloc_split_f16": (C.c_int, [C.c_void_p, C.c_void_p, C.c_void_p, C.c_size_t, C.c_float, C.c_void_p]),
     "anyloc_split_bf16": (C.c_int, [C.c_void_p, C.c_void_p, C.c_size_t, C.c_void_p]),
diff --git a/anyloc_b200/csrc/gemm_tc.cu b/anyloc_b200/csrc/gemm_tc.cu
--- a/anyloc_b200/csrc/gemm_tc.cu
+++ b/anyloc_b200/csrc/gemm_tc.cu
@@ -7,17 +7,20 @@
 
 namespace tc {
 
-constexpr int BM = 128, BN = 128;
-constexpr int KSTEPS = 4;
-constexpr int A_BYTES = BM * 128;
-constexpr int B_BYTES = BN * 128;
+constexpr int BM = 128;
 constexpr int THREADS = 384;
 constexpr int STG_BYTES = 8192;
 
-template <bool LO, bool STG = LO> struct Cfg {
+template <bool LO, bool STG = LO, int BN = 128> struct Cfg {
+  static_assert(BN == 128 || (BN == 192 && LO && STG), "192-column tiles: the staged 3-term passes");
+  static constexpr bool WIDE = BN == 192;
+  static constexpr int KB_BYTES = WIDE ? 64 : 128;
+  static constexpr int KSTEPS = KB_BYTES / 32;
+  static constexpr int A_BYTES = BM * KB_BYTES;
+  static constexpr int B_BYTES = BN * KB_BYTES;
   static constexpr int STAGE_BYTES = (LO ? 2 : 1) * (A_BYTES + B_BYTES);
   static constexpr int B_OFF = (LO ? 2 : 1) * A_BYTES;
-  static constexpr int STAGES = LO ? 3 : 6;
+  static constexpr int STAGES = WIDE ? 4 : LO ? 3 : 6;
   static constexpr int BAR_OFF = STAGES * STAGE_BYTES;
   static constexpr int SMEM_BYTES = BAR_OFF + 256 + 1024 ;
   static constexpr bool STAGED = STG;
@@ -31,11 +34,17 @@
 constexpr int CHUNK_KB_FP8 = 1;
 
 __device__ __forceinline__ void tile_coords(int tile, int num_m, int num_n, int band_n, int& m_blk, int& n_blk) {
+  if (tile >= num_m * num_n) { m_blk = num_m; n_blk = tile - num_m * num_n; return; }
   const int per_band = num_m * band_n;
   const int band = tile / per_band, r = tile - band * per_band;
   const int w = min(band_n, num_n - band * band_n);
   m_blk = r / w;
   n_blk = band * band_n + (r - m_blk * w);
+}
+
+__device__ __forceinline__ int tile_rows_rastered(int M) {
+  const int num_m = (M + BM - 1) / BM, tail = M - (num_m - 1) * BM;
+  return tail <= 64 ? num_m - 1 : num_m;
 }
 
 template <int OUT>
@@ -81,10 +90,10 @@
   }
 }
 
-template <int FMT = ANYLOC_PAIR_TF32>
+template <int FMT = ANYLOC_PAIR_TF32, int BN = 128>
 __device__ __forceinline__ void epilogue_pairs(const EpiParams& ep, int r0, int nq, int M, int N, const float* sum) {
 #pragma unroll
-  for (int j = 0; j < 16; ++j) {
+  for (int j = 0; j < BN / 8; ++j) {
     const int n = nq + j * 8;
     if (n >= N) continue;
     if (r0 < M) epi_pair<FMT>(ep, r0, n, N, sum[4 * j], sum[4 * j + 1]);
@@ -92,20 +101,21 @@
   }
 }
 
+template <int BN>
 __device__ __forceinline__ void epilogue_regs_batched(const EpiParams& ep, int r0, int nq, int M, int N, const float* sum) {
   const int mode = ep.mode;
   if (mode < 0) return;
   const int n0 = nq & ~(BN - 1);
   const bool swiglu = mode == ANYLOC_EPI_SWIGLU_SPLIT, resid = mode == ANYLOC_EPI_LS_RESID;
   if (n0 + BN > N || (!swiglu && (ep.ldo & 1))) {
-    epilogue_pairs(ep, r0, nq, M, N, sum);
+    epilogue_pairs<ANYLOC_PAIR_TF32, BN>(ep, r0, nq, M, N, sum);
     return;
   }
   const bool row0 = r0 < M, row1 = r0 + 8 < M;
   const size_t o0 = (size_t)r0 * ep.ldo, o1 = (size_t)(r0 + 8) * ep.ldo;
   const float al = ep.alpha;
 #pragma unroll
-  for (int j0 = 0; j0 < 16; j0 += 2) {
+  for (int j0 = 0; j0 < BN / 8; j0 += 2) {
     float2 b[2], g[2], ra[2], rb[2];
 #pragma unroll
     for (int jj = 0; jj < 2; ++jj) {
@@ -184,7 +194,7 @@
   tma_load_2d(smem_u32(buf), tm, smem_u32(bar), oc, m0);
 }
 
-template <int OUT, bool SWIGLU, bool RESID>
+template <int OUT, bool SWIGLU, bool RESID, int BN>
 __device__ __forceinline__ void epilogue_staged(const EpiParams& ep, const CUtensorMap* tm_out, const CUtensorMap* tm_lo,
                                                 const CUtensorMap* tm_resid, uint8_t* stg, uint64_t* rbar,
                                                 uint32_t& rphase, uint32_t& cnt, int wg, int t, int m0, int n0, int N,
@@ -203,7 +213,7 @@
     if (oc0 >= n_out) break;
     const uint32_t b = cnt & 1;
     uint8_t* buf = stg + b * STG_BYTES;
-    if (RESID) { mbar_wait(smem_u32(rbar + b), (rphase >> b) & 1); rphase ^= 1u << b; }
+    if (RESID) { mbar_wait<BN == 192>(smem_u32(rbar + b), (rphase >> b) & 1); rphase ^= 1u << b; }
 #pragma unroll
     for (int jj = 0; jj < JS; ++jj) {
       const int j = s * JS + jj, n = n0 + j * 8 + 2 * q;
@@ -260,7 +270,7 @@
   }
 }
 
-template <int FMT, int LOM>
+template <int FMT, int LOM, int BN>
 __global__ void __launch_bounds__(THREADS, 1)
 gemm_tc3_kernel(const __grid_constant__ CUtensorMap tm_a_hi, const __grid_constant__ CUtensorMap tm_a_lo,
                 const __grid_constant__ CUtensorMap tm_b_hi, const __grid_constant__ CUtensorMap tm_b_lo,
@@ -269,7 +279,8 @@
                 int M, int N, int K, int band_n, int chunk_kb, EpiParams ep) {
   constexpr bool LO = LOM != 0, has_a_lo = (LOM & 1) != 0, has_b_lo = (LOM & 2) != 0;
   static_assert(LOM == 0 || Fmt<FMT>::LO, "lo operands belong to the pair formats");
-  using C = Cfg<LO, LO || !Fmt<FMT>::LO>;
+  using C = Cfg<LO, LO || !Fmt<FMT>::LO, BN>;
+  constexpr int NACC = BN / 2;
   if (ep.gate != nullptr && *reinterpret_cast<const volatile int*>(ep.gate) == 0) return;
   extern __shared__ uint8_t smem_raw[];
   uint8_t* smem = reinterpret_cast<uint8_t*>((reinterpret_cast<uintptr_t>(smem_raw) + 1023) & ~(uintptr_t)1023);
@@ -280,7 +291,8 @@
   const int wg = threadIdx.x >> 7;
   const int num_m = (M + BM - 1) / BM, num_n = (N + BN - 1) / BN;
   const int num_tiles = num_m * num_n;
-  constexpr int BKE = 128 / (int)sizeof(typename Fmt<FMT>::T);
+  const int num_m_r = tile_rows_rastered(M);
+  constexpr int BKE = C::KB_BYTES / (int)sizeof(typename Fmt<FMT>::T);
   const int num_k = (K + BKE - 1) / BKE;
 
   if (threadIdx.x == 0) {
@@ -294,11 +306,13 @@
   __syncthreads();
 
   if (wg == 0) {
+    if constexpr (C::WIDE) setmaxnreg_dec<24>();
     if (threadIdx.x == 0) {
+      constexpr int A_BYTES = C::A_BYTES, B_BYTES = C::B_BYTES;
       const uint32_t tx_bytes = A_BYTES * (1 + ((LO && has_a_lo) ? 1 : 0)) + B_BYTES * (1 + ((LO && has_b_lo) ? 1 : 0));
       int stage = 0; uint32_t phase = 0;
       for (int tile = blockIdx.x; tile < num_tiles; tile += gridDim.x) {
-        int mb, nb; tile_coords(tile, num_m, num_n, band_n, mb, nb);
+        int mb, nb; tile_coords(tile, num_m_r, num_n, band_n, mb, nb);
         const int m0 = mb * BM, n0 = nb * BN;
         for (int kb = 0; kb < num_k; ++kb) {
           mbar_wait(smem_u32(empty_bar + stage), phase ^ 1);
@@ -316,8 +330,9 @@
     return;
   }
 
+  if constexpr (C::WIDE) setmaxnreg_inc<240>();
   const int t = threadIdx.x & 127, warp = t >> 5, lane = t & 31;
-  const uint32_t a_sub = (uint32_t)(wg - 1) * 64 * 128;
+  const uint32_t a_sub = (uint32_t)(wg - 1) * 64 * C::KB_BYTES;
   uint8_t* stg = smem + C::STG_OFF + (wg - 1) * 2 * STG_BYTES;
   uint64_t* rbar = resid_bar + (wg - 1) * 2;
   const int mode = ep.mode;
@@ -326,11 +341,19 @@
   uint32_t stg_cnt = 0, rphase = 0;
   int stage = 0; uint32_t phase = 0;
   for (int tile = blockIdx.x; tile < num_tiles; tile += gridDim.x) {
-    int mb, nb; tile_coords(tile, num_m, num_n, band_n, mb, nb);
+    int mb, nb; tile_coords(tile, num_m_r, num_n, band_n, mb, nb);
     const int m0 = mb * BM + (wg - 1) * 64, n0 = nb * BN;
-    float sum[64], acc[64];
-#pragma unroll
-    for (int j = 0; j < 64; ++j) { sum[j] = 0.f; acc[j] = 0.f; }
+    if (m0 >= M) {
+      for (int kb = 0; kb < num_k; ++kb) {
+        mbar_wait<C::WIDE>(smem_u32(full_bar + stage), phase);
+        if (t == 0) mbar_arrive(smem_u32(empty_bar + stage));
+        if (++stage == C::STAGES) { stage = 0; phase ^= 1; }
+      }
+      continue;
+    }
+    float sum[NACC], acc[NACC];
+#pragma unroll
+    for (int j = 0; j < NACC; ++j) { sum[j] = 0.f; acc[j] = 0.f; }
     int prev_stage = -1;
     for (int kb0 = 0; kb0 < num_k; kb0 += chunk_kb) {
       const int kb1 = min(num_k, kb0 + chunk_kb);
@@ -343,17 +366,18 @@
         }
       }
       for (int kb = kb0; kb < kb1; ++kb) {
-        mbar_wait(smem_u32(full_bar + stage), phase);
+        mbar_wait<C::WIDE>(smem_u32(full_bar + stage), phase);
         const uint32_t sbase = smem_u32(smem + stage * C::STAGE_BYTES);
-        const uint64_t a_hi = make_desc(sbase + a_sub), a_lo = make_desc(sbase + A_BYTES + a_sub);
-        const uint64_t b_hi = make_desc(sbase + C::B_OFF), b_lo = make_desc(sbase + C::B_OFF + B_BYTES);
+        const auto desc = [](uint32_t a) { return C::WIDE ? make_desc64(a) : make_desc(a); };
+        const uint64_t a_hi = desc(sbase + a_sub), a_lo = desc(sbase + C::A_BYTES + a_sub);
+        const uint64_t b_hi = desc(sbase + C::B_OFF), b_lo = desc(sbase + C::B_OFF + C::B_BYTES);
         wgmma_fence();
 #pragma unroll
-        for (int k = 0; k < KSTEPS; ++k) {
+        for (int k = 0; k < C::KSTEPS; ++k) {
           const uint64_t adv = (uint64_t)((k * 32) >> 4);
-          wgmma_m64n128<FMT>(acc, a_hi + adv, b_hi + adv, (kb != kb0 || k != 0) ? 1u : 0u);
-          if (has_a_lo) wgmma_m64n128<FMT>(acc, a_lo + adv, b_hi + adv, 1u);
-          if (has_b_lo) wgmma_m64n128<FMT>(acc, a_hi + adv, b_lo + adv, 1u);
+          wgmma_m64n<FMT, BN>(acc, a_hi + adv, b_hi + adv, (kb != kb0 || k != 0) ? 1u : 0u);
+          if (has_a_lo) wgmma_m64n<FMT, BN>(acc, a_lo + adv, b_hi + adv, 1u);
+          if (has_b_lo) wgmma_m64n<FMT, BN>(acc, a_hi + adv, b_lo + adv, 1u);
         }
         wgmma_commit();
         wgmma_wait<1>();
@@ -362,28 +386,28 @@
         if (++stage == C::STAGES) { stage = 0; phase ^= 1; }
       }
       wgmma_wait<0>();
-      fence_regs<64>(acc);
-#pragma unroll
-      for (int j = 0; j < 64; ++j) sum[j] += acc[j];
+      fence_regs<NACC>(acc);
+#pragma unroll
+      for (int j = 0; j < NACC; ++j) sum[j] += acc[j];
     }
     if (t == 0) mbar_arrive(smem_u32(empty_bar + prev_stage));
-    if (mode < 0 || m0 >= M) continue;
+    if (mode < 0) continue;
     if constexpr (FMT == ANYLOC_PAIR_FP8) {
       const int r = m0 + warp * 16 + (lane >> 2);
       const float s0 = r < M ? __ldg(ep.row_scale + r) : 0.f, s1 = r + 8 < M ? __ldg(ep.row_scale + r + 8) : 0.f;
 #pragma unroll
-      for (int j = 0; j < 16; ++j) { sum[4 * j] *= s0; sum[4 * j + 1] *= s0; sum[4 * j + 2] *= s1; sum[4 * j + 3] *= s1; }
+      for (int j = 0; j < BN / 8; ++j) { sum[4 * j] *= s0; sum[4 * j + 1] *= s0; sum[4 * j + 2] *= s1; sum[4 * j + 3] *= s1; }
     }
     if constexpr (!C::STAGED) {
-      epilogue_regs_batched(ep, m0 + warp * 16 + (lane >> 2), n0 + 2 * (lane & 3), M, N, sum);
+      epilogue_regs_batched<BN>(ep, m0 + warp * 16 + (lane >> 2), n0 + 2 * (lane & 3), M, N, sum);
       continue;
     }
     if (!staged) {
-      epilogue_pairs<FMT>(ep, m0 + warp * 16 + (lane >> 2), n0 + 2 * (lane & 3), M, N, sum);
+      epilogue_pairs<FMT, BN>(ep, m0 + warp * 16 + (lane >> 2), n0 + 2 * (lane & 3), M, N, sum);
       continue;
     }
 #define ANYLOC_EPI_STAGED(OUT_, SWIGLU_, RESID_)                                                                    \
-  epilogue_staged<OUT_, SWIGLU_, RESID_>(ep, &tm_out, &tm_out_lo, &tm_resid, stg, rbar, rphase, stg_cnt, wg, t, m0,  \
+  epilogue_staged<OUT_, SWIGLU_, RESID_, BN>(ep, &tm_out, &tm_out_lo, &tm_resid, stg, rbar, rphase, stg_cnt, wg, t, m0,  \
                                          n0, N, sum)
     if (mode == ANYLOC_EPI_BIAS) ANYLOC_EPI_STAGED(OUT_F32, false, false);
     else if (mode == ANYLOC_EPI_LS_RESID) ANYLOC_EPI_STAGED(OUT_F32, false, true);
@@ -428,15 +452,16 @@
   }
 }
 
-int make_map(CUtensorMap* map, const void* ptr, int rows, int K, int ld, int box_rows, int fmt) {
+int make_map(CUtensorMap* map, const void* ptr, int rows, int K, int ld, int box_rows, int fmt, int box_k_bytes) {
   EncodeTiledFn enc = get_encode();
   if (!enc) { set_error("gemm_tc: cuTensorMapEncodeTiled unavailable"); return ANYLOC_ERR_CUDA; }
   const int esz = format_info(fmt).esz;
   cuuint64_t dims[2] = {(cuuint64_t)K, (cuuint64_t)rows};
   cuuint64_t strides[1] = {(cuuint64_t)ld * esz};
-  cuuint32_t box[2] = {(cuuint32_t)(128 / esz), (cuuint32_t)box_rows};
+  cuuint32_t box[2] = {(cuuint32_t)(box_k_bytes / esz), (cuuint32_t)box_rows};
   cuuint32_t estr[2] = {1, 1};
-  CUresult r = enc(map, map_dtype(fmt), 2, (void*)ptr, dims, strides, box, estr, CU_TENSOR_MAP_INTERLEAVE_NONE, CU_TENSOR_MAP_SWIZZLE_128B,
+  CUresult r = enc(map, map_dtype(fmt), 2, (void*)ptr, dims, strides, box, estr, CU_TENSOR_MAP_INTERLEAVE_NONE,
+                   box_k_bytes == 128 ? CU_TENSOR_MAP_SWIZZLE_128B : CU_TENSOR_MAP_SWIZZLE_64B,
                    CU_TENSOR_MAP_L2_PROMOTION_L2_256B, CU_TENSOR_MAP_FLOAT_OOB_FILL_NONE);
   if (r != CUDA_SUCCESS) { set_error("gemm_tc: cuTensorMapEncodeTiled failed (%d) rows=%d K=%d ld=%d", (int)r, rows, K, ld); return ANYLOC_ERR_CUDA; }
   return ANYLOC_OK;
@@ -471,16 +496,23 @@
   return ANYLOC_OK;
 }
 
+static bool epi_split(int mode) {
+  return mode == ANYLOC_EPI_BIAS_SPLIT || mode == ANYLOC_EPI_GELU_SPLIT || mode == ANYLOC_EPI_SWIGLU_SPLIT;
+}
+static bool epi_tma_storable(const EpiParams& ep, int out, int N) {
+  const int esz = format_info(epi_split(ep.mode) ? out : ANYLOC_PAIR_TF32).esz;
+  const int n_out = ep.mode == ANYLOC_EPI_SWIGLU_SPLIT ? N / 2 : N;
+  return ((long long)ep.ldo * esz) % 16 == 0 && ((long long)n_out * esz) % 16 == 0;
+}
 static int make_epi_maps(const EpiParams& ep, int out, int M, int N, CUtensorMap* m_out, CUtensorMap* m_lo,
                          CUtensorMap* m_resid, bool* staged) {
   memset(m_out, 0, sizeof(*m_out)); memset(m_lo, 0, sizeof(*m_lo)); memset(m_resid, 0, sizeof(*m_resid));
-  const bool split = ep.mode == ANYLOC_EPI_BIAS_SPLIT || ep.mode == ANYLOC_EPI_GELU_SPLIT ||
-                     ep.mode == ANYLOC_EPI_SWIGLU_SPLIT;
+  const bool split = epi_split(ep.mode);
   const int fmt = split ? out : ANYLOC_PAIR_TF32;
   const FormatInfo& f = format_info(fmt);
   const int esz = f.esz;
   const int n_out = ep.mode == ANYLOC_EPI_SWIGLU_SPLIT ? N / 2 : N;
-  *staged = ep.mode >= 0 && ((long long)ep.ldo * esz) % 16 == 0 && ((long long)n_out * esz) % 16 == 0;
+  *staged = ep.mode >= 0 && epi_tma_storable(ep, out, N);
   if (!*staged) return ANYLOC_OK;
   const bool lo = split && f.lo;
   const int cols = STG_BYTES / STG_ROWS / (lo ? 2 : 1) / esz;
@@ -506,21 +538,22 @@
   return true;
 }
 
-static thread_local int g_last_staged = -1;
-
-template <int FMT, int LOM>
+static thread_local int g_last_staged = -1, g_last_bn = -1;
+static int g_force_bn = 0;
+
+template <int FMT, int LOM, int BN = 128>
 static int launch_impl(const void* a_hi, const void* a_lo, int lda, const void* b_hi, const void* b_lo, int ldb, int M,
                        int N, int K, const EpiParams& ep, int chunk, cudaStream_t st) {
   using namespace tc;
   constexpr bool LO = LOM != 0;
-  using CF = Cfg<LO, LO || !Fmt<FMT>::LO>;
+  using CF = Cfg<LO, LO || !Fmt<FMT>::LO, BN>;
   static_assert(CF::SMEM_BYTES_STAGED <= 232448, "GEMM over H100's shared-memory opt-in");
   CUtensorMap ma_hi, ma_lo, mb_hi, mb_lo;
   int rc;
-  if ((rc = make_map(&ma_hi, a_hi, M, K, lda, BM, FMT))) return rc;
-  if ((rc = make_map(&ma_lo, a_lo ? a_lo : a_hi, M, K, lda, BM, FMT))) return rc;
-  if ((rc = make_map(&mb_hi, b_hi, N, K, ldb, BN, FMT))) return rc;
-  if ((rc = make_map(&mb_lo, b_lo ? b_lo : b_hi, N, K, ldb, BN, FMT))) return rc;
+  if ((rc = make_map(&ma_hi, a_hi, M, K, lda, BM, FMT, CF::KB_BYTES))) return rc;
+  if ((rc = make_map(&ma_lo, a_lo ? a_lo : a_hi, M, K, lda, BM, FMT, CF::KB_BYTES))) return rc;
+  if ((rc = make_map(&mb_hi, b_hi, N, K, ldb, BN, FMT, CF::KB_BYTES))) return rc;
+  if ((rc = make_map(&mb_lo, b_lo ? b_lo : b_hi, N, K, ldb, BN, FMT, CF::KB_BYTES))) return rc;
   CUtensorMap mo, mo_lo, mr;
   bool staged = false;
   memset(&mo, 0, sizeof(mo)); memset(&mo_lo, 0, sizeof(mo_lo)); memset(&mr, 0, sizeof(mr));
@@ -528,15 +561,17 @@
   if (CF::STAGED && ep.gate == nullptr && (rc = make_epi_maps(ep, out, M, N, &mo, &mo_lo, &mr, &staged))) return rc;
   const int smem = staged ? CF::SMEM_BYTES_STAGED : CF::SMEM_BYTES;
   g_last_staged = staged ? 1 : 0;
+  g_last_bn = BN;
   static unsigned long long attr_seen = 0;
   if (first_use_on_this_device(&attr_seen)) {
-    ANYLOC_CHECK_CUDA(cudaFuncSetAttribute(gemm_tc3_kernel<FMT, LOM>, cudaFuncAttributeMaxDynamicSharedMemorySize,
+    ANYLOC_CHECK_CUDA(cudaFuncSetAttribute(gemm_tc3_kernel<FMT, LOM, BN>, cudaFuncAttributeMaxDynamicSharedMemorySize,
                                            CF::STAGED ? CF::SMEM_BYTES_STAGED : CF::SMEM_BYTES));
   }
   const int tiles = cdiv(M, BM) * cdiv(N, BN);
   const int grid = std::min(tiles, device_sm_count());
-  gemm_tc3_kernel<FMT, LOM><<<grid, THREADS, smem, st>>>(
-      ma_hi, ma_lo, mb_hi, mb_lo, mo, mo_lo, mr, staged ? 1 : 0, M, N, K, std::min(BAND_N, cdiv(N, BN)), chunk, ep);
+  gemm_tc3_kernel<FMT, LOM, BN><<<grid, THREADS, smem, st>>>(
+      ma_hi, ma_lo, mb_hi, mb_lo, mo, mo_lo, mr, staged ? 1 : 0, M, N, K, std::min(BAND_N, cdiv(N, BN)),
+      chunk * (128 / CF::KB_BYTES), ep);
   ANYLOC_CHECK_LAUNCH();
   return ANYLOC_OK;
 }
@@ -545,6 +580,23 @@
   static int chunk_env = -1;
   if (chunk_env < 0) { const char* e = getenv("ANYLOC_GEMM_CHUNK"); chunk_env = e ? atoi(e) : 0; }
   return chunk_env;
+}
+
+constexpr int WIDE_TILE_COST_PCT = 145;
+constexpr int WIDE_TILE_MIN_K = 1024;
+
+static long long tile_waves(int M, int N, int bn) {
+  const long long num_m = cdiv(M, tc::BM), num_n = cdiv(N, bn), sms = device_sm_count();
+  const bool half = M - (num_m - 1) * tc::BM <= 64;
+  const long long halves = 2 * (num_m - (half ? 1 : 0)) * num_n + (half ? num_n : 0);
+  return (halves + 2 * sms - 1) / (2 * sms);
+}
+
+static int tile_bn(const EpiParams& ep, int out, int M, int N, int K) {
+  if (ep.gate != nullptr) return 128;
+  if (g_force_bn) return g_force_bn;
+  if (ep.mode < 0 || K < WIDE_TILE_MIN_K || !tc::epi_tma_storable(ep, out, N)) return 128;
+  return tile_waves(M, N, 192) * WIDE_TILE_COST_PCT < tile_waves(M, N, 128) * 99 ? 192 : 128;
 }
 
 int gemm_tc_launch(const void* a_hi, const void* a_lo, int lda, const void* b_hi, const void* b_lo, int ldb, int M,
@@ -570,16 +622,19 @@
   const int lom = (a_lo ? 1 : 0) | (b_lo ? 2 : 0);
   const int chunk = lom == 0 ? (f16 ? tc::CHUNK_KB_COARSE : tc::CHUNK_KB_TF32)
                              : chunk_env > 0 ? chunk_env : (f16 ? tc::CHUNK_KB_F16 : tc::CHUNK_KB_TF32);
-#define ANYLOC_GEMM_LAUNCH(FMT_, LOM_) launch_impl<FMT_, LOM_>(a_hi, a_lo, lda, b_hi, b_lo, ldb, M, N, K, ep, chunk, st)
+  const bool wide = lom == 3 && tile_bn(ep_in, ep.out_fmt != ANYLOC_PAIR_TF32 ? ANYLOC_PAIR_F16 : ANYLOC_PAIR_TF32,
+                                        M, N, K) == 192;
+#define ANYLOC_GEMM_LAUNCH(FMT_, LOM_, ...) \
+  launch_impl<FMT_, LOM_, ##__VA_ARGS__>(a_hi, a_lo, lda, b_hi, b_lo, ldb, M, N, K, ep, chunk, st)
   switch (lom + (f16 ? 4 : 0)) {
     case 0: return ANYLOC_GEMM_LAUNCH(ANYLOC_PAIR_TF32, 0);
     case 1: return ANYLOC_GEMM_LAUNCH(ANYLOC_PAIR_TF32, 1);
     case 2: return ANYLOC_GEMM_LAUNCH(ANYLOC_PAIR_TF32, 2);
-    case 3: return ANYLOC_GEMM_LAUNCH(ANYLOC_PAIR_TF32, 3);
+    case 3: return wide ? ANYLOC_GEMM_LAUNCH(ANYLOC_PAIR_TF32, 3, 192) : ANYLOC_GEMM_LAUNCH(ANYLOC_PAIR_TF32, 3);
     case 4: return ANYLOC_GEMM_LAUNCH(ANYLOC_PAIR_F16, 0);
     case 5: return ANYLOC_GEMM_LAUNCH(ANYLOC_PAIR_F16, 1);
     case 6: return ANYLOC_GEMM_LAUNCH(ANYLOC_PAIR_F16, 2);
-    default: return ANYLOC_GEMM_LAUNCH(ANYLOC_PAIR_F16, 3);
+    default: return wide ? ANYLOC_GEMM_LAUNCH(ANYLOC_PAIR_F16, 3, 192) : ANYLOC_GEMM_LAUNCH(ANYLOC_PAIR_F16, 3);
   }
 #undef ANYLOC_GEMM_LAUNCH
 }
@@ -587,3 +642,9 @@
 }
 
 extern "C" int anyloc_gemm_tc_last_staged(void) { return anyloc::g_last_staged; }
+extern "C" int anyloc_gemm_tc_last_bn(void) { return anyloc::g_last_bn; }
+extern "C" int anyloc_gemm_tc_force_bn(int bn) {
+  if (bn != 0 && bn != 128 && bn != 192) return ANYLOC_ERR_ARG;
+  anyloc::g_force_bn = bn;
+  return ANYLOC_OK;
+}
diff --git a/anyloc_b200/csrc/tc_common.cuh b/anyloc_b200/csrc/tc_common.cuh
--- a/anyloc_b200/csrc/tc_common.cuh
+++ b/anyloc_b200/csrc/tc_common.cuh
@@ -16,6 +16,8 @@
 __device__ __forceinline__ void mbar_arrive(uint32_t bar) {
   asm volatile("mbarrier.arrive.shared::cta.b64 _, [%0];" ::"r"(bar) : "memory");
 }
+static __device__ __noinline__ void mbar_timeout() { __trap(); }
+template <bool TRAP_CALL = false>
 __device__ __forceinline__ void mbar_wait(uint32_t bar, uint32_t parity) {
   uint32_t done = 0;
   long long t0 = 0;
@@ -28,7 +30,10 @@
     if (!done && (it & 0x3ff) == 0x3ff) {
       long long now = clock64();
       if (t0 == 0) t0 = now;
-      else if (now - t0 > 8000000000LL) __trap();
+      else if (now - t0 > 8000000000LL) {
+        if (TRAP_CALL) mbar_timeout();
+        else __trap();
+      }
     }
   }
 }
@@ -59,6 +64,15 @@
   d |= (uint64_t)1 << 16;
   d |= (uint64_t)(1024 >> 4) << 32;
   d |= (uint64_t)1 << 62;
+  return d;
+}
+
+__device__ __forceinline__ uint64_t make_desc64(uint32_t saddr) {
+  uint64_t d = 0;
+  d |= (uint64_t)((saddr & 0x3FFFF) >> 4);
+  d |= (uint64_t)1 << 16;
+  d |= (uint64_t)(512 >> 4) << 32;
+  d |= (uint64_t)2 << 62;
   return d;
 }
 
@@ -102,6 +116,47 @@
 #undef ANYLOC_WG_D64
 #undef ANYLOC_WG_D64_STR
 
+#define ANYLOC_WG_D96                                                                                               \
+  "+f"(d[0]), "+f"(d[1]), "+f"(d[2]), "+f"(d[3]), "+f"(d[4]), "+f"(d[5]), "+f"(d[6]), "+f"(d[7]), "+f"(d[8]),       \
+      "+f"(d[9]), "+f"(d[10]), "+f"(d[11]), "+f"(d[12]), "+f"(d[13]), "+f"(d[14]), "+f"(d[15]), "+f"(d[16]),        \
+      "+f"(d[17]), "+f"(d[18]), "+f"(d[19]), "+f"(d[20]), "+f"(d[21]), "+f"(d[22]), "+f"(d[23]), "+f"(d[24]),       \
+      "+f"(d[25]), "+f"(d[26]), "+f"(d[27]), "+f"(d[28]), "+f"(d[29]), "+f"(d[30]), "+f"(d[31]), "+f"(d[32]),       \
+      "+f"(d[33]), "+f"(d[34]), "+f"(d[35]), "+f"(d[36]), "+f"(d[37]), "+f"(d[38]), "+f"(d[39]), "+f"(d[40]),       \
+      "+f"(d[41]), "+f"(d[42]), "+f"(d[43]), "+f"(d[44]), "+f"(d[45]), "+f"(d[46]), "+f"(d[47]), "+f"(d[48]),       \
+      "+f"(d[49]), "+f"(d[50]), "+f"(d[51]), "+f"(d[52]), "+f"(d[53]), "+f"(d[54]), "+f"(d[55]), "+f"(d[56]),       \
+      "+f"(d[57]), "+f"(d[58]), "+f"(d[59]), "+f"(d[60]), "+f"(d[61]), "+f"(d[62]), "+f"(d[63]), "+f"(d[64]),       \
+      "+f"(d[65]), "+f"(d[66]), "+f"(d[67]), "+f"(d[68]), "+f"(d[69]), "+f"(d[70]), "+f"(d[71]), "+f"(d[72]),       \
+      "+f"(d[73]), "+f"(d[74]), "+f"(d[75]), "+f"(d[76]), "+f"(d[77]), "+f"(d[78]), "+f"(d[79]), "+f"(d[80]),       \
+      "+f"(d[81]), "+f"(d[82]), "+f"(d[83]), "+f"(d[84]), "+f"(d[85]), "+f"(d[86]), "+f"(d[87]), "+f"(d[88]),       \
+      "+f"(d[89]), "+f"(d[90]), "+f"(d[91]), "+f"(d[92]), "+f"(d[93]), "+f"(d[94]), "+f"(d[95])
+#define ANYLOC_WG_D96_STR                                                                                           \
+  "{%0, %1, %2, %3, %4, %5, %6, %7, %8, %9, %10, %11, %12, %13, %14, %15, %16, %17, %18, %19, %20, %21, %22, %23, " \
+  "%24, %25, %26, %27, %28, %29, %30, %31, %32, %33, %34, %35, %36, %37, %38, %39, %40, %41, %42, %43, %44, %45, "  \
+  "%46, %47, %48, %49, %50, %51, %52, %53, %54, %55, %56, %57, %58, %59, %60, %61, %62, %63, %64, %65, %66, %67, "  \
+  "%68, %69, %70, %71, %72, %73, %74, %75, %76, %77, %78, %79, %80, %81, %82, %83, %84, %85, %86, %87, %88, %89, "  \
+  "%90, %91, %92, %93, %94, %95}"
+#define ANYLOC_WG_M64N192(SHAPE_TYPES, TAIL)                                                                        \
+  asm volatile("{\n\t.reg .pred p;\n\tsetp.ne.b32 p, %98, 0;\n\t"                                                 \
+               "wgmma.mma_async.sync.aligned.m64n192" SHAPE_TYPES " " ANYLOC_WG_D96_STR ", %96, %97, p, 1, 1" TAIL     \
+               ";\n\t}"                                                                                              \
+               : ANYLOC_WG_D96 : "l"(adesc), "l"(bdesc), "r"(scale_d))
+
+template <int FMT>
+__device__ __forceinline__ void wgmma_m64n192(float* d, uint64_t adesc, uint64_t bdesc, uint32_t scale_d) {
+  static_assert(FMT == ANYLOC_PAIR_TF32 || FMT == ANYLOC_PAIR_F16, "192-column tiles: the 3-term pair formats");
+  if constexpr (FMT == ANYLOC_PAIR_TF32) ANYLOC_WG_M64N192("k8.f32.tf32.tf32", "");
+  else ANYLOC_WG_M64N192("k16.f32.f16.f16", ", 0, 0");
+}
+#undef ANYLOC_WG_M64N192
+#undef ANYLOC_WG_D96
+#undef ANYLOC_WG_D96_STR
+
+template <int FMT, int BN>
+__device__ __forceinline__ void wgmma_m64n(float* d, uint64_t adesc, uint64_t bdesc, uint32_t scale_d) {
+  if constexpr (BN == 192) wgmma_m64n192<FMT>(d, adesc, bdesc, scale_d);
+  else wgmma_m64n128<FMT>(d, adesc, bdesc, scale_d);
+}
+
 __device__ __forceinline__ void tma_load_3d(uint32_t dst, const CUtensorMap* map, uint32_t bar, int c0, int c1, int c2) {
   asm volatile(
       "cp.async.bulk.tensor.3d.shared::cluster.global.mbarrier::complete_tx::bytes [%0], [%1, {%3, %4, %5}], [%2];"
@@ -157,7 +212,7 @@
 #undef ANYLOC_WG_D32
 #undef ANYLOC_WG_D32_STR
 
-int make_map(CUtensorMap* map, const void* ptr, int rows, int K, int ld, int box_rows, int fmt);
+int make_map(CUtensorMap* map, const void* ptr, int rows, int K, int ld, int box_rows, int fmt, int box_k_bytes = 128);
 int make_map_3d16(CUtensorMap* map, const void* ptr, int imgs, int rows, int cols, int box_rows, int fmt);
 
 }
diff --git a/include/anyloc_b200.h b/include/anyloc_b200.h
--- a/include/anyloc_b200.h
+++ b/include/anyloc_b200.h
@@ -197,6 +197,8 @@
                    const float* gamma, const float* resid, void* out, void* out_lo, int ldo, int out_dtype,
                    int engine, void* stream);
 int anyloc_gemm_tc_last_staged(void);
+int anyloc_gemm_tc_last_bn(void);
+int anyloc_gemm_tc_force_bn(int bn);
 int anyloc_split_tf32(const float* x, float* hi, float* lo, size_t n, void* stream);
 int anyloc_split_f16(const float* x, void* hi, void* lo, size_t n, float scale, void* stream);
 int anyloc_split_bf16(const float* x, void* y, size_t n, void* stream);
```

After: 181.8, median of 6. 1.01x the previous value.
